# VictoriaMetrics/VictoriaLogs

Hardware: NVIDIA H100
Metric: log rows scanned/sec (LogsQL phrase+regex) (higher is better)
Workload: dtype u8

## Files before the change

### victorialogs_b200/csrc/vl_engine.cu

```cuda
#include <dlfcn.h>
#include <algorithm>
#include <atomic>
#include <chrono>
#include <cmath>
#include <limits>
#include <thread>
#include <cstdio>
#include <cstdlib>
#include <cstring>
#include <functional>
#include <map>
#include <memory>
#include <mutex>
#include "vl_copier.h"
#include "vl_engine.h"
#include "vl_kernels.cuh"
#include "vl_program.h"
#include "vl_part.h"
#include "vl_mathnum.cuh"

using namespace vl;

namespace vl {
static thread_local std::string g_thread_err;
void set_thread_error(const std::string& s) { g_thread_err = s; }
}

struct vlscan_program {
    Program p;
    struct Image { DevBuf leaves, prepass, regexes, blob, u64s, u32s; DevProgram view; };
    std::map<int, std::unique_ptr<Image>> images;
    std::mutex mu;
    const DevProgram& image(int device, cudaStream_t st) {
        std::lock_guard<std::mutex> g(mu);
        auto it = images.find(device);
        if (it != images.end()) return it->second->view;
        auto im = std::make_unique<Image>();
        auto up = [&](DevBuf& b, const void* src, size_t n) { b.ensure(std::max<size_t>(n, 16)); if (n) VL_CUDA(cudaMemcpyAsync(b.p, src, n, cudaMemcpyHostToDevice, st)); };
        up(im->leaves, p.leaves.data(), p.leaves.size() * sizeof(DevLeaf));
        up(im->prepass, p.prepass.data(), p.prepass.size() * sizeof(DevPrepass));
        up(im->regexes, p.regexes.data(), p.regexes.size() * sizeof(DevRegex));
        up(im->blob, p.blob.data(), p.blob.size());
        up(im->u64s, p.u64s.data(), p.u64s.size() * 8);
        up(im->u32s, p.u32s.data(), p.u32s.size() * 4);
        VL_CUDA(cudaStreamSynchronize(st));
        im->view = DevProgram{im->leaves.as<DevLeaf>(), im->prepass.as<DevPrepass>(), im->regexes.as<DevRegex>(), im->blob.as<uint8_t>(), im->u64s.as<uint64_t>(), im->u32s.as<uint32_t>()};
        auto& ref = *im;
        images[device] = std::move(im);
        return ref.view;
    }
    ~vlscan_program() { for (auto& kv : images) { cudaSetDevice(kv.first); kv.second->leaves.release(); kv.second->prepass.release(); kv.second->regexes.release(); kv.second->blob.release(); kv.second->u64s.release(); kv.second->u32s.release(); } }
};

struct vlscan_host_blocks {
    void* pinned = nullptr; size_t bytes = 0;
    std::vector<vlscan_block> blocks;
    std::vector<vlscan_column> cols;
    std::vector<std::string> fields;
    std::vector<std::vector<uint32_t>> dict_offsets;
    std::vector<std::unique_ptr<std::vector<uint8_t>>> owned;
    std::vector<uint64_t> source;
};
struct vlscan_part { vl::part::PartReader r; };

void* vlscan_ctx::ensure_pinned(size_t n) {
    if (n <= pinned_cap) return pinned;
    if (pinned) cudaFreeHost(pinned);
    pinned = nullptr; pinned_cap = 0;
    VL_CUDA(cudaMallocHost(&pinned, n));
    pinned_cap = n;
    return pinned;
}

namespace {

struct ZstdWriter {
    size_t (*compress)(void*, size_t, const void*, size_t, int) = nullptr;
    size_t (*bound)(size_t) = nullptr;
    unsigned (*is_error)(size_t) = nullptr;
    bool ok = false;
    ZstdWriter() {
        void* h = dlopen("libzstd.so.1", RTLD_NOW | RTLD_GLOBAL);
        if (!h) return;
        compress = (decltype(compress))dlsym(h, "ZSTD_compress");
        bound = (decltype(bound))dlsym(h, "ZSTD_compressBound");
        is_error = (decltype(is_error))dlsym(h, "ZSTD_isError");
        ok = compress && bound && is_error;
    }
};
ZstdWriter& zstd_writer() { static ZstdWriter z; return z; }

}

namespace vl {
void finish_batch_layout(vlscan_ctx* ctx, vlscan_batch* b, const std::vector<uint32_t>& rows) {
    b->nblocks = rows.size();
    b->h_rows = rows;
    b->h_word_off.assign(rows.size() + 1, 0);
    b->rows = 0;
    for (size_t i = 0; i < rows.size(); i++) { b->h_word_off[i + 1] = b->h_word_off[i] + (rows[i] + 63) / 64; b->rows += rows[i]; }
    b->nwords = b->h_word_off.back();
    std::vector<uint32_t> wb(b->nwords);
    std::vector<uint64_t> init(b->nwords);
    for (size_t i = 0; i < rows.size(); i++) {
        for (uint64_t w = b->h_word_off[i]; w < b->h_word_off[i + 1]; w++) { wb[w] = (uint32_t)i; init[w] = ~0ull; }
        uint32_t tail = rows[i] & 63;
        if (tail) init[b->h_word_off[i + 1] - 1] = (~0ull) >> (64 - tail);
    }
    b->blk_rows.ensure(std::max<size_t>(rows.size() * 4, 16));
    b->blk_word_off.ensure((rows.size() + 1) * 8);
    b->word_block.ensure(std::max<size_t>(b->nwords * 4, 16));
    b->init_bitmap.ensure(std::max<size_t>(b->nwords * 8, 16));
    if (!rows.empty()) VL_CUDA(cudaMemcpyAsync(b->blk_rows.p, rows.data(), rows.size() * 4, cudaMemcpyHostToDevice, ctx->stream));
    VL_CUDA(cudaMemcpyAsync(b->blk_word_off.p, b->h_word_off.data(), (rows.size() + 1) * 8, cudaMemcpyHostToDevice, ctx->stream));
    if (b->nwords) {
        VL_CUDA(cudaMemcpyAsync(b->word_block.p, wb.data(), b->nwords * 4, cudaMemcpyHostToDevice, ctx->stream));
        VL_CUDA(cudaMemcpyAsync(b->init_bitmap.p, init.data(), b->nwords * 8, cudaMemcpyHostToDevice, ctx->stream));
    }
    VL_CUDA(cudaStreamSynchronize(ctx->stream));
}
}

static uint64_t collect_values_blocks(const vlscan_block* blocks, uint64_t nblocks, std::vector<ZValuesBlock>& zv, const uint8_t* need = nullptr, uint32_t nfields = 0, std::vector<size_t>* at = nullptr) {
    uint64_t zc = 512;
    if (at) at->assign((size_t)nblocks * nfields, SIZE_MAX);
    for (uint64_t b = 0; b < nblocks; b++)
        for (uint32_t k = 0; k < blocks[b].ncols; k++) {
            const vlscan_column& c = blocks[b].cols[k];
            if (c.kind != VLSCAN_COL_VALUES || c.stage != VLSCAN_STAGE_ONDISK) continue;
            if (need && (c.field >= nfields || !need[b * nfields + c.field])) continue;
            if (at && c.field < nfields && (*at)[b * nfields + c.field] == SIZE_MAX) (*at)[b * nfields + c.field] = zv.size();
            zv.push_back({c.values, (size_t)c.values_len, zc});
            zc += c.values_len;
        }
    return zc;
}
static double now_s() { return std::chrono::duration<double>(std::chrono::steady_clock::now().time_since_epoch()).count(); }

namespace {
struct Upload {
    vlscan_ctx* ctx; vlscan_batch* out; const vlscan_block* blocks; uint64_t nblocks; uint32_t nfields; vlscan_stats* stats;
    const std::vector<char>* need_bloom;
    std::vector<DevColumn>& cols = out->h_cols;
    const bool dbg = getenv("VLSCAN_DEBUG_TIMING") != nullptr; const double t_start = now_s();
    Copier io{ctx};
    std::vector<uint32_t> rows = std::vector<uint32_t>(nblocks);
    std::vector<Piece> pieces;
    std::vector<std::unique_ptr<std::vector<uint8_t>>> owned;
    uint64_t cursor = 16;
    ZstdJob zjob;
    uint64_t regen_cursor = 0;
    struct Ondisk { uint64_t col; uint32_t lens_frame, data_frame; uint64_t lens_rel, data_rel; };
    std::vector<Ondisk> ondisk;
    std::vector<OndiskCol> ocols;
    struct TsFrame { uint64_t block; uint32_t frame; uint64_t rel; };
    std::vector<TsFrame> ts_frames;
    std::vector<DevTimestamps> tsv;
    std::vector<ZValuesBlock> zv; std::vector<ZValuesInfo> zinfo; std::vector<size_t> zv_of; std::vector<uint64_t> ts_zoff; size_t zbad = SIZE_MAX; std::string zmsg;
    uint64_t add_piece(const uint8_t* src, uint64_t len) { uint64_t off = arena_reserve(cursor, len); if (len) pieces.push_back({src, len, off}); return off; }
    template <class F> void walk(bool ts, F&& f) {
        for (uint64_t b = 0; b < nblocks; b++) {
            const vlscan_block& blk = blocks[b];
            if (blk.rows > (8u << 20)) throw BadInput("block rows exceed maxRowsPerBlock (8Mi)");
            rows[b] = (uint32_t)blk.rows;
            if (ts) timestamps(blk, b);
            for (uint32_t k = 0; k < blk.ncols; k++) {
                if (blk.cols[k].field >= nfields) throw BadInput("column refers to a field outside the batch field table");
                f(blk, blk.cols[k], (size_t)b * nfields + blk.cols[k].field);
            }
        }
    }
    void sources(const uint8_t* need, bool ts) {
        uint64_t zc = collect_values_blocks(blocks, nblocks, zv, need, nfields, &zv_of);
        for (const ZValuesBlock& v : zv) if (v.n) io.src.push_back({v.p, v.n, v.zoff});
        ts_zoff.resize(ts ? nblocks : 0);
        for (uint64_t b = 0; b < nblocks && ts; b++) {
            const vlscan_block& blk = blocks[b];
            if (blk.ts_marshal_type != MT_ZSTD_NEAREST_DELTA2 && blk.ts_marshal_type != MT_ZSTD_NEAREST_DELTA) continue;
            if (blk.timestamps_len > vl::part::kMaxTimestampsBlockSize) throw BadInput("timestamps block size cannot exceed 8 MiB");
            ts_zoff[b] = zc;
            if (blk.timestamps_len) io.src.push_back({blk.timestamps, blk.timestamps_len, zc});
            zc += blk.timestamps_len;
        }
        if (!io.src.empty()) { ctx->zsrc.ensure(zc + 512); io.send_sources(ctx->zsrc.as<uint8_t>()); }
        zinfo.resize(zv.size());
        const double t_w = now_s();
        if (!zv.empty()) zjob.add_values_blocks(zv.data(), zv.size(), host_threads(), zinfo.data(), &zbad, &zmsg);
        if (dbg) fprintf(stderr, "[vlscan upload] header walk of %zu values blocks on %d host threads: %.1f ms (after %.1f ms of collecting and enqueueing the copies)\n",
                         zv.size(), host_threads(), 1e3 * (now_s() - t_w), 1e3 * (t_w - t_start));
    }
    template <class F> void header(const vlscan_column& c, size_t i, F&& payload) {
        DevColumn& d = cols[i];
        if (d.kind != COL_MISSING) throw BadInput("duplicate column for one field in a block");
        if (c.kind == VLSCAN_COL_CONST) {
            d.kind = COL_CONST; d.meta_len = (uint32_t)c.const_len; d.meta_off = add_piece(c.const_value, c.const_len);
            return;
        }
        if (c.kind != VLSCAN_COL_VALUES) throw BadInput("unknown column kind");
        if (c.value_type < VT_STRING || c.value_type >= VT_MAX) throw BadInput("unknown valueType");
        d.kind = COL_VALUES; d.vt = c.value_type; d.min_value = c.min_value; d.max_value = c.max_value;
        payload();
        if (c.bloom_len % 8) throw BadInput("cannot unmarshal bloomFilter from src with size not multiple by 8");
        if (need_bloom && !(*need_bloom)[c.field]) { d.bloom_words = 0; d.bloom_off = add_piece(c.bloom, 0); }
        else { d.bloom_words = (uint32_t)(c.bloom_len / 8); d.bloom_off = add_piece(c.bloom, c.bloom_len); }
        if (c.value_type == VT_DICT) {
            if (c.dict_len > 8) throw BadInput("valuesDict may contain max 8 items");
            d.dict_len = c.dict_len;
            uint32_t total = c.dict_len ? c.dict_offsets[c.dict_len] : 0;
            d.meta_len = total;
            if (c.dict_len && c.dict_blob == (const uint8_t*)c.dict_offsets + 4 * (c.dict_len + 1)) {
                d.meta_off = add_piece((const uint8_t*)c.dict_offsets, 4 * (c.dict_len + 1) + total);
            } else {
                auto meta = std::make_unique<std::vector<uint8_t>>();
                meta->resize(4 * (c.dict_len + 1) + total);
                if (c.dict_len) memcpy(meta->data(), c.dict_offsets, 4 * (c.dict_len + 1)); else memset(meta->data(), 0, 4);
                if (total) memcpy(meta->data() + 4 * (c.dict_len + 1), c.dict_blob, total);
                d.meta_off = add_piece(meta->data(), meta->size());
                owned.push_back(std::move(meta));
            }
        }
    }
    void values(const vlscan_block& blk, const vlscan_column& c, size_t ci) {
        DevColumn& d = cols[ci];
        if (c.stage == VLSCAN_STAGE_ONDISK) {
            const size_t z = zv_of[ci];
            if (z >= zbad) throw BadInput(zmsg);
            const uint64_t lens_len = zinfo[z].lens_len, data_len = zinfo[z].data_len;
            if (data_len > 0xFFFFFFFFull) throw BadInput("values block too large");
            const uint64_t lr = arena_reserve(regen_cursor, lens_len + 15), dr = arena_reserve(regen_cursor, data_len);
            d.lens_off = lr + 16; d.data_off = dr; d.data_len = data_len;
            ondisk.push_back({ci, (uint32_t)(2 * z), (uint32_t)(2 * z + 1), lr + 15, dr});
            ocols.push_back({ci, lens_len, blk.rows});
        } else if (c.stage == VLSCAN_STAGE_DECODED) {
            const uint8_t* lens_items = c.lens_items; const uint64_t lens_len = c.lens_items_len, data_len = c.data_len;
            if (lens_len < 1) throw BadInput("cannot unmarshal uint64 block type from empty src");
            uint8_t lt = lens_items[0];
            if (lt > 7) throw BadInput("unexpected uint64 block type");
            uint64_t want = lt < 4 ? (blk.rows << lt) : (1ull << (lt - 4));
            if (lens_len - 1 != want) throw BadInput("unexpected block length for uint items");
            d.lens_type = lt;
            if (lt >= 4) { uint64_t v = 0; for (uint64_t i = 0; i < want; i++) v = (v << 8) | lens_items[1 + i]; if (v > 0xFFFFFFFFull) throw BadInput("row length does not fit 32 bits"); d.lens_const = (uint32_t)v; }
            if (data_len > 0xFFFFFFFFull) throw BadInput("values block too large");
            d.lens_off = add_piece(lens_items + 1, lens_len - 1);
            d.data_off = add_piece(c.data, data_len); d.data_len = data_len;
            d.data_const = (blk.rows >= 2 && lt >= 4 && data_len == d.lens_const) ? 1 : 0;
        } else throw BadInput("unknown values stage");
    }
    void timestamps(const vlscan_block& blk, uint64_t b) {
        if (!blk.ts_marshal_type) return;
        if (blk.ts_marshal_type > MT_NEAREST_DELTA) throw BadInput("unknown MarshalType of a timestamps block");
        if (blk.timestamps_len > vl::part::kMaxTimestampsBlockSize) throw BadInput("timestamps block size cannot exceed 8 MiB");
        if (tsv.empty()) { tsv.resize(nblocks); memset(tsv.data(), 0, nblocks * sizeof(DevTimestamps)); }
        DevTimestamps& t = tsv[b];
        t.first = blk.min_timestamp; t.max = blk.max_timestamp;
        if (blk.ts_marshal_type == MT_ZSTD_NEAREST_DELTA2 || blk.ts_marshal_type == MT_ZSTD_NEAREST_DELTA) {
            uint64_t regen = 0; uint32_t id = 0;
            zjob.add_frame(blk.timestamps, blk.timestamps_len, ts_zoff[b], &regen, &id);
            if (regen > 10ull * blk.rows + 16) throw BadInput("cannot unmarshal timestamps: the decompressed block is larger than its varints can be");
            t.mt = blk.ts_marshal_type == MT_ZSTD_NEAREST_DELTA2 ? MT_NEAREST_DELTA2 : MT_NEAREST_DELTA;
            t.len = (uint32_t)regen;
            ts_frames.push_back({b, id, arena_reserve(regen_cursor, regen)});
        } else {
            t.mt = (uint8_t)blk.ts_marshal_type; t.len = (uint32_t)blk.timestamps_len;
            t.off = add_piece(blk.timestamps, blk.timestamps_len);
        }
    }

    uint64_t commit(DevBuf& region, const std::vector<uint64_t>* patch, bool layout) {
        const uint64_t regen_base = (cursor + kArenaAlign - 1) / kArenaAlign * kArenaAlign;
        for (const Ondisk& o : ondisk) {
            DevColumn& d = cols[o.col];
            d.lens_off += regen_base; d.data_off += regen_base;
            zjob.set_dst(o.lens_frame, regen_base + o.lens_rel); zjob.set_dst(o.data_frame, regen_base + o.data_rel);
        }
        for (const TsFrame& tf : ts_frames) { tsv[tf.block].off = regen_base + tf.rel; zjob.set_dst(tf.frame, regen_base + tf.rel); }
        const bool have_z = !ondisk.empty() || !ts_frames.empty();
        if (have_z) cursor = regen_base + regen_cursor;
        const uint64_t bytes = cursor + kArenaPad;
        const double t_desc = now_s();
        region.ensure(bytes);
        const double t_alloc = now_s();
        uint8_t* cols_base = region.as<uint8_t>();
        std::vector<ColPatch> patches;
        if (patch) {
            const uint64_t delta = (uint64_t)(uintptr_t)region.p - (uint64_t)(uintptr_t)out->arena.p;
            cols_base = out->arena.as<uint8_t>();
            patches.resize(patch->size());
            for (size_t i = 0; i < patch->size(); i++) {
                DevColumn& d = cols[(*patch)[i]];
                d.lens_off += delta; d.data_off += delta;
                patches[i].col = (*patch)[i]; patches[i].c = d;
            }
        }
        cudaStream_t cs = ctx->copy_stream;
        cudaEvent_t ev_cleared = io.events.make(), ev_copied = io.events.make();
        VL_CUDA(cudaMemsetAsync(region.p, 0, bytes, ctx->stream));
        VL_CUDA(cudaEventRecord(ev_cleared, ctx->stream));
        VL_CUDA(cudaStreamWaitEvent(cs, ev_cleared, 0));
        const double t_h2d = dbg ? now_s() : 0;
        double t_zrun = 0;
        if (have_z) {
            zjob.set_group_hook([&](uint64_t src_end) { io.wait_sources(ctx->stream, src_end); });
            zjob.run(ctx, ctx->zsrc.as<uint8_t>(), region.as<uint8_t>());
            io.ship_sources(UINT64_MAX);
            if (dbg) t_zrun = now_s();
        }
        io.copy(pieces, region.as<uint8_t>());
        DevBuf& table = patch ? ctx->patch : out->cols;
        const void* entries = patch ? (const void*)patches.data() : (const void*)cols.data();
        const size_t table_bytes = patch ? patches.size() * sizeof(ColPatch) : cols.size() * sizeof(DevColumn);
        table.ensure(std::max<size_t>(table_bytes, 16));
        if (table_bytes) VL_CUDA(cudaMemcpyAsync(table.p, entries, table_bytes, cudaMemcpyHostToDevice, cs));
        io.h2d += table_bytes;
        if (!patch) out->has_ts = !tsv.empty();
        if (!tsv.empty()) {
            out->ts.ensure(nblocks * sizeof(DevTimestamps));
            VL_CUDA(cudaMemcpyAsync(out->ts.p, tsv.data(), nblocks * sizeof(DevTimestamps), cudaMemcpyHostToDevice, cs));
            io.h2d += nblocks * sizeof(DevTimestamps);
        }
        VL_CUDA(cudaEventRecord(ev_copied, cs));
        if (!patches.empty()) {
            VL_CUDA(cudaStreamWaitEvent(ctx->stream, ev_copied, 0));
            k_patch_cols<<<cdiv(patches.size(), 128), 128, 0, ctx->stream>>>(out->cols.as<DevColumn>(), ctx->patch.as<ColPatch>(), (uint32_t)patches.size());
            launch_check(ctx);
        }
        const double t_enq = dbg ? now_s() : 0;
        if (have_z) {
            VL_CUDA(cudaStreamWaitEvent(ctx->stream, ev_copied, 0));
            ctx->zcols.ensure(16 + ocols.size() * sizeof(OndiskCol));
            VL_CUDA(cudaMemsetAsync(ctx->zcols.p, 0, 16, ctx->stream));
            VL_CUDA(cudaMemcpyAsync(ctx->zcols.as<uint8_t>() + 16, ocols.data(), ocols.size() * sizeof(OndiskCol), cudaMemcpyHostToDevice, ctx->stream));
            if (!ocols.empty()) {
                k_finish_ondisk_cols<<<cdiv(ocols.size(), 128), 128, 0, ctx->stream>>>(cols_base, out->cols.as<DevColumn>(), (const OndiskCol*)(ctx->zcols.as<uint8_t>() + 16),
                                                                                         (uint32_t)ocols.size(), ctx->zcols.as<unsigned long long>());
                launch_check(ctx);
            }
            io.h2d += ocols.size() * sizeof(OndiskCol);
            zjob.check(ctx);
            unsigned long long cst[2] = {0, 0};
            VL_CUDA(cudaMemcpy(cst, ctx->zcols.p, 16, cudaMemcpyDeviceToHost));
            static const char* what[] = {"", "cannot unmarshal uint64 block type from empty src", "unexpected uint64 block type", "unexpected block length for uint items", "row length does not fit 32 bits"};
            if (cst[0]) throw BadInput(what[std::min<unsigned long long>(cst[0], 4)]);
        }
        VL_CUDA(cudaStreamWaitEvent(ctx->stream, ev_copied, 0));
        double t_copy = 0;
        if (dbg) { VL_CUDA(cudaStreamSynchronize(ctx->stream)); t_copy = now_s(); }
        if (nfields) out->note_columns(cols);
        if (layout) finish_batch_layout(ctx, out, rows);
        else VL_CUDA(cudaStreamSynchronize(ctx->stream));
        if (dbg) fprintf(stderr, "[vlscan upload] blocks=%llu arena=%.1f MB h2d=%.1f MB pieces=%zu+%zu pinned=%d: describe %.1f ms, alloc %.1f ms, copy %.1f ms (%.1f GB/s), "
                                 "zstd %llu frames / %llu blocks / %llu sequences: enqueue %.1f ms, decode %.1f ms; layout %.1f ms\n", (unsigned long long)nblocks,
                         bytes / 1e6, io.h2d / 1e6, pieces.size(), io.src.size(), (int)io.all_pinned, 1e3 * (t_desc - t_start), 1e3 * (t_alloc - t_desc), 1e3 * (t_enq - (t_zrun > 0 ? t_zrun : t_h2d)), io.h2d / 1e9 / std::max(t_copy - t_start, 1e-9),
                         (unsigned long long)zjob.frames(), (unsigned long long)zjob.compressed_blocks(), (unsigned long long)zjob.sequences(), 1e3 * (t_zrun > 0 ? t_zrun - t_h2d : 0), 1e3 * (t_copy - t_enq), 1e3 * (now_s() - t_copy));
        if (layout) io.h2d += out->nwords * 12 + nblocks * 12;
        if (stats) stats->h2d_bytes += io.h2d;
        return bytes;
    }
};
}

enum UploadMode { UP_FULL = 0, UP_HEADERS = 1, UP_VALUES = 2, UP_LATE = 3 };
static void do_upload(vlscan_ctx* ctx, const char* const* field_names, const size_t* field_name_lens, uint32_t nfields, const vlscan_block* blocks,
                      uint64_t nblocks, vlscan_batch* out, vlscan_stats* stats, const std::vector<char>* need_bloom = nullptr, UploadMode mode = UP_FULL,
                      const uint8_t* need = nullptr, uint64_t* zframes = nullptr) {
    VL_CUDA(cudaSetDevice(ctx->device));
    if (nblocks > 0xFFFFFFF0ull) throw BadInput("too many blocks in one batch");
    out->device = ctx->device; out->nfields = nfields;
    Upload u{ctx, out, blocks, nblocks, nfields, stats, need_bloom};
    if (mode == UP_FULL || mode == UP_HEADERS) {
        for (uint32_t f = 0; f < nfields; f++) out->field_names.emplace_back(field_names[f], field_name_lens[f]);
        u.cols.assign((size_t)nblocks * std::max<uint32_t>(nfields, 1), DevColumn{});
        memset(u.cols.data(), 0, u.cols.size() * sizeof(DevColumn));
        out->late_used = 0; out->split_hdr = mode == UP_HEADERS;
    } else if (u.cols.size() != (size_t)nblocks * std::max<uint32_t>(nfields, 1) || !need) throw BadInput("internal: values phase of a bloom-first upload without its header phase");
    try {
        switch (mode) {
        case UP_FULL:
            u.sources(nullptr, true);
            u.walk(true, [&](const vlscan_block& blk, const vlscan_column& c, size_t i) { u.header(c, i, [&] { u.values(blk, c, i); }); });
            out->arena_bytes = u.commit(out->arena, nullptr, true);
            out->harena_bytes = 0;
            std::vector<DevColumn>().swap(out->h_cols);
            break;
        case UP_HEADERS:
            u.walk(false, [&](const vlscan_block&, const vlscan_column& c, size_t i) {
                u.header(c, i, [&] {
                    if (c.stage != VLSCAN_STAGE_ONDISK && c.stage != VLSCAN_STAGE_DECODED) throw BadInput("unknown values stage");
                    u.cols[i].values_state = VALUES_DEFERRED;
                });
            });
            out->harena_bytes = u.commit(out->harena, nullptr, true);
            break;
        case UP_VALUES:
            u.sources(need, true);
            u.walk(true, [&](const vlscan_block& blk, const vlscan_column& c, size_t i) {
                if (c.kind != VLSCAN_COL_VALUES) return;
                u.cols[i].values_state = need[i] ? VALUES_STAGED : VALUES_ABSENT;
                if (need[i]) u.values(blk, c, i);
            });
            out->arena_bytes = u.commit(out->arena, nullptr, false);
            break;
        case UP_LATE: {
            std::vector<uint64_t> staged;
            u.sources(need, false);
            u.walk(false, [&](const vlscan_block& blk, const vlscan_column& c, size_t i) {
                if (c.kind != VLSCAN_COL_VALUES || !need[i]) return;
                if (u.cols[i].values_state == VALUES_STAGED) throw BadInput("duplicate column for one field in a block");
                u.cols[i].values_state = VALUES_STAGED;
                u.values(blk, c, i);
                staged.push_back(i);
            });
            if (out->late_used == out->late.size()) out->late.emplace_back();
            u.commit(out->late[out->late_used], &staged, false);
            out->late_used++;
            *zframes += u.zjob.frames();
            break;
        }
        }
    } catch (...) {
        cudaStreamSynchronize(ctx->copy_stream); cudaStreamSynchronize(ctx->stream);
        throw;
    }
}

const uint32_t* vl::row_offsets(vlscan_ctx* ctx, const BatchView& B, int slot, const uint32_t* list, const uint32_t* wc, unsigned long long* stats, int wc_slot) {
    uint8_t* ready = ctx->ready[slot].as<uint8_t>();
    if (!ctx->ready_cleared[slot]) { VL_CUDA(cudaMemsetAsync(ready, 0, B.nblocks, ctx->stream)); ctx->ready_cleared[slot] = 1; }
    k_lens_offsets<<<ctx->sm_count * 8, 256, 0, ctx->stream>>>(B, slot, list, wc, ctx->row_off8[slot].as<uint32_t>(), ready, stats, wc_slot); launch_check(ctx);
    return ctx->row_off8[slot].as<uint32_t>();
}

namespace {
struct ScanRun {
    vlscan_ctx* ctx; const vlscan_program* prog; const vlscan_batch* batch;
    DevProgram P; BatchView B; std::vector<int> field_slot;
    unsigned long long* stats;
    size_t regs_used = 0;

    uint64_t* new_reg() {
        if (regs_used == ctx->regs.size()) ctx->regs.emplace_back();
        DevBuf& r = ctx->regs[regs_used++];
        r.ensure(std::max<size_t>(B.nwords * 8, 16));
        return r.as<uint64_t>();
    }
    void free_reg() { regs_used--; }
    void copy_reg(uint64_t* dst, const uint64_t* src) { if (B.nwords) VL_CUDA(cudaMemcpyAsync(dst, src, B.nwords * 8, cudaMemcpyDeviceToDevice, ctx->stream)); }
    void andnot(uint64_t* a, const uint64_t* b) { if (!B.nwords) return; k_andnot<<<cdiv(B.nwords, 256), 256, 0, ctx->stream>>>(a, b, B.nwords); launch_check(ctx); }
    void prepass(const PNode& nd, uint64_t* reg) {
        if (nd.prepass_count == 0) return;
        std::vector<int> slots(nd.prepass_count);
        for (int e = 0; e < nd.prepass_count; e++) slots[e] = field_slot[prog->p.prepass[nd.prepass_begin + e].field];
        size_t off = slots_cursor; slots_cursor += slots.size();
        ctx->slots.ensure(std::max<size_t>(slots_total * 4, 16));
        VL_CUDA(cudaMemcpyAsync(ctx->slots.as<int>() + off, slots.data(), slots.size() * 4, cudaMemcpyHostToDevice, ctx->stream));
        k_prepass<<<cdiv((uint64_t)B.nblocks * 32, 128), 128, 0, ctx->stream>>>(P, B, (uint32_t)nd.prepass_begin, (uint32_t)nd.prepass_count, ctx->slots.as<int>() + off,
                                                                             nd.kind == F_OR, reg, stats);
        launch_check(ctx);
    }
    size_t slots_cursor = 0, slots_total = 0;

    void leaf(int leaf_idx, uint64_t* reg) {
        const DevLeaf& L = prog->p.leaves[leaf_idx];
        if (L.kind == F_NOOP) return;
        int slot = L.field >= 0 ? field_slot[L.field] : -1;
        uint8_t* action = ctx->action.as<uint8_t>(); uint64_t* payload = ctx->payload.as<uint64_t>(); uint64_t* leaf_bm = ctx->leaf_bm.as<uint64_t>();
        uint32_t* lens_blocks = ctx->lens_blocks.as<uint32_t>(); uint32_t* row_blocks = ctx->row_blocks.as<uint32_t>(); uint32_t* wc = ctx->work_count.as<uint32_t>();
        ScanTile* tiles = ctx->tiles.as<ScanTile>();
        VL_CUDA(cudaMemsetAsync(wc, 0, WC_COUNT * 4, ctx->stream));
        if (L.kind == F_EQ_FIELD || L.kind == F_LE_FIELD) {
            const int slot_b = field_slot[L.field2];
            uint32_t* lens_b = ctx->lens_blocks2.as<uint32_t>();
            k_plan_pair<<<cdiv((uint64_t)B.nblocks * 32, 256), 256, 0, ctx->stream>>>(P, B, (uint32_t)leaf_idx, slot, slot_b, reg, action, payload, lens_blocks, lens_b, row_blocks, wc, stats);
            launch_check(ctx);
            if (B.nwords) {
                const int persistent = ctx->sm_count * 8;
                const uint32_t *ro_a = nullptr, *ro_b = nullptr;
                for (int side = 0; side < 2; side++) {
                    const int sl = side ? slot_b : slot;
                    if (sl >= 0) (side ? ro_b : ro_a) = row_offsets(ctx, B, sl, side ? lens_b : lens_blocks, wc, stats, side ? WC_LENS2 : WC_LENS);
                }
                k_row_pair<<<persistent, 256, 0, ctx->stream>>>(P, B, (uint32_t)leaf_idx, slot, slot_b, row_blocks, wc, payload, reg, ro_a, ro_b, leaf_bm, stats); launch_check(ctx);
                k_apply_leaf<<<cdiv(B.nwords, 256), 256, 0, ctx->stream>>>(B, action, leaf_bm, reg); launch_check(ctx);
            }
            return;
        }
        k_plan_leaf<<<cdiv(B.nblocks, VL_PLAN_WARPS), VL_PLAN_WARPS * 32, 0, ctx->stream>>>(P, B, (uint32_t)leaf_idx, slot, reg, action, payload, lens_blocks, row_blocks, tiles, wc, stats);
        launch_check(ctx);
        if (slot >= 0 && B.nwords) {
            const uint32_t vts = batch->slot_vt_mask.empty() ? ~0u : batch->slot_vt_mask[slot];
            const bool has_string = vts >> VT_STRING & 1, has_dict = vts >> VT_DICT & 1;
            const bool has_numeric = (vts & ~((1u << VT_STRING) | (1u << VT_DICT))) != 0;
            const bool may_scan = L.str_strategy == STR_SCAN && has_string;
            const bool may_row = (has_string && L.str_strategy != STR_ALL) || has_numeric;
            const uint32_t* ro = may_scan || may_row ? row_offsets(ctx, B, slot, lens_blocks, wc, stats, WC_LENS) : nullptr;
            if (may_scan) {
                VL_CUDA(cudaMemsetAsync(leaf_bm, 0, B.nwords * 8, ctx->stream));
                ScanParams sp; memset(&sp, 0, sizeof sp);
                sp.mode = L.scan_mode; sp.needle_off = L.scan_needle_off; sp.needle_len = L.scan_needle_len; sp.starts_tok = L.starts_tok; sp.ends_tok = L.ends_tok; sp.regex = L.regex;
                const bool masked = fill_scan_patterns(prog->p.blob.data() + L.scan_needle_off, L.scan_needle_len, sp.pat, sp.msk, sp.delta, sp.nd16);
                if (L.scan_mode == SCAN_CONTAINS || L.scan_mode >= SCAN_RX_DOTPLUS) { sp.starts_tok = sp.ends_tok = 0; }
                auto& evp = next_scan_events();
                VL_CUDA(cudaEventRecord(evp.first, ctx->stream));
                if (masked) k_substr_scan<true><<<ctx->sm_count * ctx->scan_occ[1], VL_SCAN_THREADS, 0, ctx->stream>>>(P, B, slot, sp, tiles, wc, ro, leaf_bm);
                else k_substr_scan<false><<<ctx->sm_count * ctx->scan_occ[0], VL_SCAN_THREADS, 0, ctx->stream>>>(P, B, slot, sp, tiles, wc, ro, leaf_bm);
                launch_check(ctx);
                VL_CUDA(cudaEventRecord(evp.second, ctx->stream));
            }
            if (may_row) { k_row_match<<<ctx->sm_count * ctx->row_occ, 256, 0, ctx->stream>>>(P, B, (uint32_t)leaf_idx, slot, row_blocks, wc, action, payload, reg, ro, leaf_bm); launch_check(ctx); }
            if (has_dict || has_numeric) { k_word_match<<<cdiv(B.nwords, 128), 128, 0, ctx->stream>>>(P, B, (uint32_t)leaf_idx, slot, action, payload, reg, leaf_bm, stats); launch_check(ctx); }
        }
        if (L.kind == F_TIME && B.nwords) {
            ctx->ts_vals.ensure(B.nwords * 64 * 8);
            k_time_match<<<ctx->sm_count * 4, 256, 0, ctx->stream>>>(B, (long long)L.aux0, (long long)L.aux1, row_blocks, wc, ctx->ts_vals.as<unsigned long long>(), leaf_bm, stats);
            launch_check(ctx);
        }
        if (B.nwords) { k_apply_leaf<<<cdiv(B.nwords, 256), 256, 0, ctx->stream>>>(B, action, leaf_bm, reg); launch_check(ctx); }
    }
    std::pair<cudaEvent_t, cudaEvent_t>& next_scan_events() {
        if (ctx->scan_events_used == ctx->scan_events.size()) { cudaEvent_t a, b; VL_CUDA(cudaEventCreate(&a)); VL_CUDA(cudaEventCreate(&b)); ctx->scan_events.emplace_back(a, b); }
        return ctx->scan_events[ctx->scan_events_used++];
    }
    void probe_leaf(int leaf_idx, const uint64_t* reg, uint8_t* need) {
        const DevLeaf& L = prog->p.leaves[leaf_idx];
        if (L.kind == F_NOOP || L.kind == F_TIME) return;
        const int slot = L.field >= 0 ? field_slot[L.field] : -1;
        if (L.kind == F_EQ_FIELD || L.kind == F_LE_FIELD) {
            k_plan_pair<<<cdiv((uint64_t)B.nblocks * 32, 256), 256, 0, ctx->stream>>>(P, B, (uint32_t)leaf_idx, slot, field_slot[L.field2], reg, nullptr, nullptr, nullptr, nullptr, nullptr, nullptr, stats, need);
        } else {
            if (slot < 0) return;
            k_plan_leaf<<<cdiv(B.nblocks, VL_PLAN_WARPS), VL_PLAN_WARPS * 32, 0, ctx->stream>>>(P, B, (uint32_t)leaf_idx, slot, reg, nullptr, nullptr, nullptr, nullptr, nullptr, nullptr, stats, need);
        }
        launch_check(ctx);
    }
    void probe_node(int id, uint64_t* reg, uint8_t* need) {
        const PNode& nd = prog->p.nodes[id];
        switch (nd.kind) {
        case F_NOOP: break;
        case F_AND: case F_OR: {
            uint64_t* r = reg;
            if (nd.prepass_count) { r = new_reg(); copy_reg(r, reg); prepass(nd, r); }
            for (int k : nd.kids) probe_node(k, r, need);
            if (nd.prepass_count) free_reg();
            break;
        }
        case F_NOT: probe_node(nd.kids[0], reg, need); break;
        default: probe_leaf(nd.leaf, reg, need);
        }
    }
    void node(int id, uint64_t* reg) {
        const PNode& nd = prog->p.nodes[id];
        switch (nd.kind) {
        case F_NOOP: break;
        case F_AND: prepass(nd, reg); for (int k : nd.kids) node(k, reg); break;
        case F_OR: {
            prepass(nd, reg);
            uint64_t* res = new_reg(); uint64_t* tmp = new_reg();
            copy_reg(res, reg);
            for (int k : nd.kids) { copy_reg(tmp, res); node(k, tmp); andnot(res, tmp); }
            andnot(reg, res);
            free_reg(); free_reg();
            break;
        }
        case F_NOT: { uint64_t* tmp = new_reg(); copy_reg(tmp, reg); node(nd.kids[0], tmp); andnot(reg, tmp); free_reg(); break; }
        default: leaf(nd.leaf, reg);
        }
    }
};
}

static void read_stats(vlscan_ctx* ctx, vlscan_stats* st, bool check_error) {
    unsigned long long h[ST_COUNT];
    VL_CUDA(cudaMemcpyAsync(h, ctx->stats.p, sizeof h, cudaMemcpyDeviceToHost, ctx->stream));
    VL_CUDA(cudaStreamSynchronize(ctx->stream));
    if (check_error && h[ST_ERROR]) {
        static const char* const msg[] = {"", "cannot unmarshal strings: row lengths do not add up to the data length", "too big index for dict value",
                                          "unexpected length for binary representation of a number", "", "", "the filter needs the timestamps of a block that was handed over without them", "cannot unmarshal timestamps",
                                          "internal: a filter reached the values of a column that the bloom-first probe pass had left on the host"};
        throw BadInput(msg[std::min<unsigned long long>(h[ST_ERROR], 8)]);
    }
    if (!st) return;
    st->values_bytes += h[ST_VALUES_BYTES]; st->bloom_probe_bytes += h[ST_BLOOM_BYTES]; st->columns_read += h[ST_COLUMNS_READ];
    st->bitmap_bytes += h[ST_BITMAP_BYTES]; st->rows_matched += h[ST_ROWS_MATCHED]; st->blocks_matched += h[ST_BLOCKS_MATCHED];
    st->scan_kernel_bytes += h[ST_SCAN_BYTES];
    float ms = 0;
    VL_CUDA(cudaEventElapsedTime(&ms, ctx->ev_begin, ctx->ev_end)); st->gpu_ms += ms;
    for (size_t i = 0; i < ctx->scan_events_used; i++) { VL_CUDA(cudaEventElapsedTime(&ms, ctx->scan_events[i].first, ctx->scan_events[i].second)); st->scan_kernel_ms += ms; }
}

static void do_scan(vlscan_ctx* ctx, const vlscan_program* prog, const vlscan_batch* batch, vlscan_stats* stats) {
    VL_CUDA(cudaSetDevice(ctx->device));
    if (batch->device != ctx->device) throw BadInput("batch lives on another device than the ctx");
    ScanRun run{ctx, prog, batch};
    run.P = const_cast<vlscan_program*>(prog)->image(ctx->device, ctx->stream);
    run.B = batch->view();
    const Program& pr = prog->p;
    run.field_slot.assign(pr.fields.size(), -1);
    for (size_t f = 0; f < pr.fields.size(); f++) for (uint32_t s = 0; s < batch->nfields; s++) if (batch->field_names[s] == pr.fields[f]) run.field_slot[f] = (int)s;
    for (auto& nd : pr.nodes) run.slots_total += nd.prepass_count;
    uint64_t nb = std::max<uint64_t>(batch->nblocks, 1), nw = std::max<uint64_t>(batch->nwords, 1);
    ctx->action.ensure(nb); ctx->payload.ensure(nb * 8); ctx->leaf_bm.ensure(nw * 8);
    ctx->lens_blocks.ensure(nb * 4); ctx->lens_blocks2.ensure(nb * 4); ctx->row_blocks.ensure(nb * 4); ctx->work_count.ensure(WC_COUNT * 4);
    {
        uint64_t max_tiles = batch->arena_bytes / VL_TILE_BYTES + nb + 16;
        ctx->tiles.ensure(max_tiles * sizeof(ScanTile));
    }
    ctx->stats.ensure(ST_COUNT * 8); ctx->totals.ensure(32); ctx->counts.ensure(nb * 4);
    if (ctx->row_off8.size() < batch->nfields) { ctx->row_off8.resize(batch->nfields); ctx->ready.resize(batch->nfields); }
    ctx->ready_cleared.assign(batch->nfields, 0);
    for (uint32_t s = 0; s < batch->nfields; s++) { ctx->row_off8[s].ensure(nw * 32); ctx->ready[s].ensure(nb); }
    uint64_t launches0 = ctx->launches;
    ctx->scan_events_used = 0;
    run.stats = ctx->stats.as<unsigned long long>();
    VL_CUDA(cudaEventRecord(ctx->ev_begin, ctx->stream));
    VL_CUDA(cudaMemsetAsync(ctx->stats.p, 0, ST_COUNT * 8, ctx->stream));
    VL_CUDA(cudaMemsetAsync(ctx->totals.p, 0, 32, ctx->stream));
    uint64_t* reg = run.new_reg();
    run.copy_reg(reg, batch->init_bitmap.as<uint64_t>());
    if (batch->nblocks) {
        run.node(pr.root, reg);
        k_finalize<<<cdiv(batch->nblocks, 8), 256, 0, ctx->stream>>>(run.B, reg, ctx->counts.as<uint32_t>(), run.stats, ctx->totals.as<unsigned long long>());
        launch_check(ctx);
    }
    VL_CUDA(cudaEventRecord(ctx->ev_end, ctx->stream));
    ctx->last_batch = batch; ctx->has_result = true; ctx->kept = false; ctx->last_launches = ctx->launches - launches0;
    ctx->last_nblocks = batch->nblocks; ctx->last_nwords = batch->nwords; ctx->last_rows = batch->rows;
    if (stats) {
        read_stats(ctx, stats, true);
        stats->blocks += batch->nblocks; stats->rows += batch->rows; stats->gpu_launches += ctx->launches - launches0;
    }
}

static void do_probe(vlscan_ctx* ctx, const vlscan_program* prog, const vlscan_batch* batch, std::vector<uint8_t>& need) {
    VL_CUDA(cudaSetDevice(ctx->device));
    ScanRun run{ctx, prog, batch};
    run.P = const_cast<vlscan_program*>(prog)->image(ctx->device, ctx->stream);
    run.B = batch->view();
    const Program& pr = prog->p;
    run.field_slot.assign(pr.fields.size(), -1);
    for (size_t f = 0; f < pr.fields.size(); f++) for (uint32_t s = 0; s < batch->nfields; s++) if (batch->field_names[s] == pr.fields[f]) run.field_slot[f] = (int)s;
    for (auto& nd : pr.nodes) run.slots_total += nd.prepass_count;
    const size_t cells = (size_t)batch->nblocks * batch->nfields;
    need.assign(cells, 0);
    if (!cells || !batch->nwords) return;
    ctx->need.ensure(std::max<size_t>(cells, 16)); ctx->stats.ensure(ST_COUNT * 8);
    VL_CUDA(cudaMemsetAsync(ctx->need.p, 0, cells, ctx->stream));
    VL_CUDA(cudaMemsetAsync(ctx->stats.p, 0, ST_COUNT * 8, ctx->stream));
    run.stats = ctx->stats.as<unsigned long long>();
    uint64_t* reg = run.new_reg();
    run.copy_reg(reg, batch->init_bitmap.as<uint64_t>());
    run.probe_node(pr.root, reg, ctx->need.as<uint8_t>());
    VL_CUDA(cudaMemcpyAsync(need.data(), ctx->need.p, cells, cudaMemcpyDeviceToHost, ctx->stream));
    VL_CUDA(cudaStreamSynchronize(ctx->stream));
}

extern "C" {

int vlscan_device_count(void) {
    int n = 0;
    if (cudaGetDeviceCount(&n) != cudaSuccess) { cudaGetLastError(); return 0; }
    return n;
}

vlscan_ctx* vlscan_ctx_create(int device) {
    vlscan_ctx* ctx = new vlscan_ctx();
    int rc = guarded(nullptr, [&] {
        int n = vlscan_device_count();
        if (n <= 0) throw CudaFail("no CUDA device is available: libvlscan has no CPU fallback", 100);
        ctx->device = ((device % n) + n) % n;
        VL_CUDA(cudaSetDevice(ctx->device));
        VL_CUDA(cudaStreamCreateWithFlags(&ctx->stream, cudaStreamNonBlocking));
        VL_CUDA(cudaStreamCreateWithFlags(&ctx->copy_stream, cudaStreamNonBlocking));
        VL_CUDA(cudaEventCreate(&ctx->ev_begin)); VL_CUDA(cudaEventCreate(&ctx->ev_end));
        cudaDeviceProp prop; VL_CUDA(cudaGetDeviceProperties(&prop, ctx->device)); ctx->sm_count = prop.multiProcessorCount;
        VL_CUDA(cudaOccupancyMaxActiveBlocksPerMultiprocessor(&ctx->scan_occ[0], k_substr_scan<false>, VL_SCAN_THREADS, 0));
        VL_CUDA(cudaOccupancyMaxActiveBlocksPerMultiprocessor(&ctx->scan_occ[1], k_substr_scan<true>, VL_SCAN_THREADS, 0));
        for (int& o : ctx->scan_occ) o = std::max(o, 1);
        VL_CUDA(cudaOccupancyMaxActiveBlocksPerMultiprocessor(&ctx->row_occ, k_row_match, 256, 0));
        ctx->row_occ = std::max(ctx->row_occ, 1);
    });
    if (rc) { delete ctx; return nullptr; }
    return ctx;
}
void vlscan_ctx_free(vlscan_ctx* ctx) {
    if (!ctx) return;
    cudaSetDevice(ctx->device);
    if (ctx->copy_stream) cudaStreamSynchronize(ctx->copy_stream);
    if (ctx->stream) cudaStreamSynchronize(ctx->stream);
    for (DevBuf* b : {&ctx->action, &ctx->payload, &ctx->leaf_bm, &ctx->lens_blocks, &ctx->row_blocks, &ctx->work_count, &ctx->stats, &ctx->totals, &ctx->counts, &ctx->slots, &ctx->hit_offs, &ctx->hits, &ctx->tiles, &ctx->lens_blocks2}) b->release();
    for (auto& r : ctx->regs) r.release();
    for (auto& r : ctx->row_off8) r.release();
    for (auto& r : ctx->ready) r.release();
    ctx->zsrc.release(); ctx->zcols.release(); ctx->ztest.release(); ctx->ts_vals.release();
    for (DevBuf* b : {&ctx->hit_block, &ctx->glens, &ctx->goffs, &ctx->gtiles, &ctx->gout, &ctx->gstat, &ctx->hslot, &ctx->hblk, &ctx->htab, &ctx->hgrp, &ctx->lcand, &ctx->ftab, &ctx->patch, &ctx->unstaged}) b->release();
    for (DevBuf& b : ctx->ftxt) b.release();
    zstd_dev_free(ctx->zdev);
    delete ctx->pool;
    if (ctx->pinned) cudaFreeHost(ctx->pinned);
    delete ctx->recycle;
    for (auto& e : ctx->scan_events) { cudaEventDestroy(e.first); cudaEventDestroy(e.second); }
    if (ctx->ev_begin) cudaEventDestroy(ctx->ev_begin);
    if (ctx->ev_end) cudaEventDestroy(ctx->ev_end);
    if (ctx->copy_stream) cudaStreamDestroy(ctx->copy_stream);
    if (ctx->stream) cudaStreamDestroy(ctx->stream);
    delete ctx;
}
const char* vlscan_last_error(const vlscan_ctx* ctx) { return ctx ? ctx->err.c_str() : g_thread_err.c_str(); }
void* vlscan_ctx_stream(const vlscan_ctx* ctx) { return (void*)ctx->stream; }
int vlscan_ctx_sync(vlscan_ctx* ctx) { return guarded(ctx, [&] { VL_CUDA(cudaSetDevice(ctx->device)); VL_CUDA(cudaStreamSynchronize(ctx->stream)); }); }

int vlscan_program_create(const void* tree, size_t tree_len, vlscan_program** out) {
    *out = nullptr;
    auto* pg = new vlscan_program();
    int rc = guarded(nullptr, [&] { ProgramBuilder(tree, tree_len, pg->p).build(); });
    if (rc) { delete pg; return rc; }
    *out = pg;
    return 0;
}
void vlscan_program_free(vlscan_program* prog) { delete prog; }
uint32_t vlscan_program_nfields(const vlscan_program* prog) { return (uint32_t)prog->p.fields.size(); }
const char* vlscan_program_field(const vlscan_program* prog, uint32_t i, size_t* len) { if (i >= prog->p.fields.size()) { *len = 0; return nullptr; } *len = prog->p.fields[i].size(); return prog->p.fields[i].data(); }
int64_t vlscan_program_leaf_tokens(const vlscan_program* prog, uint32_t leaf, char* buf, size_t cap) {
    if (leaf >= prog->p.leaf_tokens.size()) return -1;
    std::string s; for (size_t i = 0; i < prog->p.leaf_tokens[leaf].size(); i++) { if (i) s.push_back('\n'); s += prog->p.leaf_tokens[leaf][i]; }
    if (s.size() > cap) return -1;
    memcpy(buf, s.data(), s.size());
    return (int64_t)s.size();
}

int vlscan_eval_predicate(int kind, const void* value, size_t value_len, const void* arg1, size_t arg1_len, const void* arg2, size_t arg2_len, uint64_t aux0, uint64_t aux1) {
    if (value_len > 0xFFFFFFFFull || arg1_len > 0xFFFFFFFFull || arg2_len > 0xFFFFFFFFull) return -1;
    const uint8_t* v = (const uint8_t*)value; const uint32_t vn = (uint32_t)value_len;
    const uint8_t* a = (const uint8_t*)arg1; const uint32_t an = (uint32_t)arg1_len;
    switch (kind) {
    case F_REGEXP: {
        try { return vl::compile_regex(std::string((const char*)a, an)).match(v, vn) ? 1 : 0; } catch (const vl::RxError& e) { vl::set_thread_error(e.what()); return -2; }
    }
    case 14: return vl::any_case_match(v, vn, a, an, false) ? 1 : 0;
    case 15: return vl::any_case_match(v, vn, a, an, true) ? 1 : 0;
    case 16: return vl::match_sequence(v, vn, vl::PhraseList{a, an}) ? 1 : 0;
    case 17: return vl::match_all_phrases(v, vn, vl::PhraseList{a, an}) ? 1 : 0;
    case 18: return vl::match_any_phrase(v, vn, vl::PhraseList{a, an}) ? 1 : 0;
    }
    if (kind < F_EXACT_PREFIX || kind > F_IPV4_RANGE) return -1;
    return vl::range_predicate(kind, (const uint8_t*)value, (uint32_t)value_len, (const uint8_t*)arg1, (uint32_t)arg1_len, (const uint8_t*)arg2, (uint32_t)arg2_len, aux0, aux1) ? 1 : 0;
}

int64_t vlscan_program_prepass_tokens(const vlscan_program* prog, char* buf, size_t cap) {
    const Program& P = prog->p;
    std::string s;
    for (const PNode& nd : P.nodes) {
        if (nd.kind != F_AND && nd.kind != F_OR) continue;
        s += nd.kind == F_AND ? "A" : "O";
        for (int k = 0; k < nd.prepass_count; k++) {
            const DevPrepass& pp = P.prepass[(size_t)nd.prepass_begin + k];
            s += "\t" + P.fields[pp.field];
            const uint32_t* offs = (const uint32_t*)(P.blob.data() + pp.tok_offs_off);
            for (uint32_t t = 0; t < pp.ntokens; t++) { s += "\x1f"; s.append((const char*)P.blob.data() + pp.tok_blob_off + offs[t], offs[t + 1] - offs[t]); }
        }
        s += "\n";
    }
    if (s.size() > cap) return -1;
    memcpy(buf, s.data(), s.size());
    return (int64_t)s.size();
}

int64_t vlscan_program_in_hashes(const vlscan_program* prog, uint32_t leaf, uint64_t* out, size_t cap) {
    const Program& P = prog->p;
    if (leaf >= P.leaves.size() || P.leaves[leaf].kind != F_IN) return -1;
    const DevLeaf& L = P.leaves[leaf];
    std::vector<uint64_t> v;
    v.push_back(L.nhashes); v.insert(v.end(), P.u64s.begin() + L.hashes_off, P.u64s.begin() + L.hashes_off + L.nhashes);
    if (L.in_skip_sets) v.push_back(UINT64_MAX);
    else {
        v.push_back(L.in_nsets);
        for (uint32_t k = 0; k < L.in_nsets; k++) {
            const uint32_t off = P.u32s[L.in_sets_off + 2 * k], n = P.u32s[L.in_sets_off + 2 * k + 1];
            v.push_back(n); v.insert(v.end(), P.u64s.begin() + off, P.u64s.begin() + off + n);
        }
    }
    if (v.size() > cap) return -1;
    memcpy(out, v.data(), v.size() * 8);
    return (int64_t)v.size();
}

int64_t vlscan_program_in_typed(const vlscan_program* prog, uint32_t leaf, int value_type, uint64_t* out, size_t cap) {
    const Program& P = prog->p;
    if (leaf >= P.leaves.size() || P.leaves[leaf].kind != F_IN || value_type < VT_UINT8 || value_type >= VT_MAX) return -1;
    const DevLeaf& L = P.leaves[leaf];
    const uint32_t n = L.in_typed_cnt[value_type];
    if (n > cap) return -1;
    if (n) memcpy(out, P.u64s.data() + L.in_typed_off[value_type], (size_t)n * 8);
    return (int64_t)n;
}

int vlscan_parse_typed(int value_type, const void* s, size_t len, uint64_t* out) {
    const std::string v((const char*)s, len);
    uint64_t u = 0; int64_t i = 0; double f = 0; uint32_t ip = 0;
    switch (value_type) {
    case VT_UINT8: case VT_UINT16: case VT_UINT32: case VT_UINT64: if (!vl::parse_u64(v, &u)) return 0; *out = u; return 1;
    case VT_INT64: if (!vl::parse_i64(v, &i)) return 0; *out = (uint64_t)i; return 1;
    case VT_FLOAT64: if (!vl::parse_f64_exact(v, &f)) return 0; memcpy(out, &f, 8); return 1;
    case VT_IPV4: if (!vl::parse_ipv4(v, &ip)) return 0; *out = ip; return 1;
    case VT_ISO8601: if (!vl::parse_iso8601(v, &i)) return 0; *out = (uint64_t)i; return 1;
    }
    return -1;
}

double vlscan_parse_math_number(const void* s, size_t len) {
    if (len > 0xFFFFFFFFull) return NAN;
    return vl::mn::parse_math_number((const uint8_t*)s, (uint32_t)len);
}

int vlscan_format_float64(uint64_t ieee_bits, char* buf, size_t cap) {
    uint8_t tmp[VL_FMT_F64_MAX];
    int n = vl::fmt_f64(tmp, ieee_bits);
    if ((size_t)n > cap) return -1;
    memcpy(buf, tmp, (size_t)n);
    return n;
}

int vlscan_batch_upload(vlscan_ctx* ctx, const char* const* field_names, const size_t* field_name_lens, uint32_t nfields, const vlscan_block* blocks,
                        uint64_t nblocks, vlscan_batch** out, vlscan_stats* stats) {
    *out = nullptr;
    auto* b = new vlscan_batch();
    int rc = guarded(ctx, [&] { do_upload(ctx, field_names, field_name_lens, nfields, blocks, nblocks, b, stats); });
    if (rc) { delete b; return rc; }
    *out = b;
    return 0;
}
void vlscan_batch_free(vlscan_batch* batch) { delete batch; }
uint64_t vlscan_batch_nblocks(const vlscan_batch* b) { return b->nblocks; }
uint64_t vlscan_batch_rows(const vlscan_batch* b) { return b->rows; }
uint64_t vlscan_batch_words(const vlscan_batch* b) { return b->nwords; }
uint64_t vlscan_batch_device_bytes(const vlscan_batch* b) { return b->device_bytes(); }

int vlscan_batch_download(vlscan_ctx* ctx, const vlscan_batch* batch, vlscan_host_blocks** out) {
    *out = nullptr;
    auto* hb = new vlscan_host_blocks();
    int rc = guarded(ctx, [&] {
        VL_CUDA(cudaSetDevice(ctx->device));
        if (batch->split_hdr) throw BadInput("a batch staged bloom-first cannot be downloaded");
        hb->bytes = batch->arena_bytes;
        VL_CUDA(cudaMallocHost(&hb->pinned, std::max<size_t>(hb->bytes, 16)));
        std::vector<DevColumn> cols((size_t)batch->nblocks * batch->nfields);
        VL_CUDA(cudaMemcpyAsync(hb->pinned, batch->arena.p, hb->bytes, cudaMemcpyDeviceToHost, ctx->stream));
        if (!cols.empty()) VL_CUDA(cudaMemcpyAsync(cols.data(), batch->cols.p, cols.size() * sizeof(DevColumn), cudaMemcpyDeviceToHost, ctx->stream));
        VL_CUDA(cudaStreamSynchronize(ctx->stream));
        hb->fields = batch->field_names;
        const uint8_t* base = (const uint8_t*)hb->pinned;
        hb->blocks.resize(batch->nblocks);
        hb->cols.reserve(cols.size());
        std::vector<size_t> first(batch->nblocks + 1, 0);
        for (uint64_t b = 0; b < batch->nblocks; b++) {
            first[b] = hb->cols.size();
            for (uint32_t f = 0; f < batch->nfields; f++) {
                const DevColumn& d = cols[(size_t)b * batch->nfields + f];
                if (d.kind == COL_MISSING) continue;
                vlscan_column c; memset(&c, 0, sizeof c);
                c.field = f;
                if (d.kind == COL_CONST) { c.kind = VLSCAN_COL_CONST; c.const_value = base + d.meta_off; c.const_len = d.meta_len; hb->cols.push_back(c); continue; }
                c.kind = VLSCAN_COL_VALUES; c.value_type = d.vt; c.stage = VLSCAN_STAGE_DECODED; c.dict_len = d.dict_len; c.min_value = d.min_value; c.max_value = d.max_value;
                uint64_t items = d.lens_type < 4 ? ((uint64_t)batch->h_rows[b] << d.lens_type) : (1ull << (d.lens_type - 4));
                uint8_t* tb = (uint8_t*)hb->pinned + d.lens_off - 1;
                *tb = d.lens_type;
                c.lens_items = tb; c.lens_items_len = items + 1;
                c.data = base + d.data_off; c.data_len = d.data_len;
                c.bloom = base + d.bloom_off; c.bloom_len = (uint64_t)d.bloom_words * 8;
                if (d.vt == VT_DICT) { c.dict_offsets = (const uint32_t*)(base + d.meta_off); c.dict_blob = base + d.meta_off + 4 * (d.dict_len + 1); }
                hb->cols.push_back(c);
            }
        }
        first[batch->nblocks] = hb->cols.size();
        for (uint64_t b = 0; b < batch->nblocks; b++) { hb->blocks[b].rows = batch->h_rows[b]; hb->blocks[b].ncols = (uint32_t)(first[b + 1] - first[b]); hb->blocks[b].cols = hb->cols.data() + first[b]; }
        if (batch->has_ts && batch->nblocks) {
            std::vector<DevTimestamps> ts(batch->nblocks);
            VL_CUDA(cudaMemcpy(ts.data(), batch->ts.p, ts.size() * sizeof(DevTimestamps), cudaMemcpyDeviceToHost));
            for (uint64_t b = 0; b < batch->nblocks; b++) {
                if (!ts[b].mt) continue;
                vlscan_block& blk = hb->blocks[b];
                blk.ts_marshal_type = ts[b].mt; blk.timestamps = base + ts[b].off; blk.timestamps_len = ts[b].len;
                blk.min_timestamp = ts[b].first; blk.max_timestamp = ts[b].max;
            }
        }
    });
    if (rc) { if (hb->pinned) cudaFreeHost(hb->pinned); delete hb; return rc; }
    *out = hb;
    return 0;
}
static void marshal_bytes_block(std::vector<uint8_t>& dst, const uint8_t* src, size_t n) {
    if (n < 128) { dst.push_back(0); dst.push_back((uint8_t)n); dst.insert(dst.end(), src, src + n); return; }
    ZstdWriter& z = zstd_writer();
    if (!z.ok) throw BadInput("libzstd.so.1 is not available for compressing values blocks");
    int level = n <= 512 ? 1 : n <= 4096 ? 2 : 3;
    size_t cap = z.bound(n), old = dst.size();
    dst.push_back(1);
    dst.resize(old + 1 + 10 + cap);
    size_t got = z.compress(dst.data() + old + 11, cap, src, n, level);
    if (z.is_error(got)) throw BadInput("ZSTD_compress failed");
    uint8_t vu[10]; int k = 0; uint64_t v = got; while (v >= 0x80) { vu[k++] = (uint8_t)(v | 0x80); v >>= 7; } vu[k++] = (uint8_t)v;
    memcpy(dst.data() + old + 1, vu, k);
    memmove(dst.data() + old + 1 + k, dst.data() + old + 11, got);
    dst.resize(old + 1 + k + got);
}

int vlscan_host_blocks_compress(const vlscan_host_blocks* in, int threads, vlscan_host_blocks** out) {
    *out = nullptr;
    auto* hb = new vlscan_host_blocks();
    int rc = guarded(nullptr, [&] {
        const size_t ncols = in->cols.size();
        std::vector<std::vector<uint8_t>> packed(ncols);
        std::atomic<size_t> next{0}; std::atomic<bool> failed{false}; std::string fail_msg; std::mutex mu;
        auto work = [&] {
            for (;;) {
                size_t i0 = next.fetch_add(64); if (i0 >= ncols || failed) return;
                for (size_t i = i0; i < std::min(ncols, i0 + 64); i++) {
                    const vlscan_column& c = in->cols[i];
                    if (c.kind != VLSCAN_COL_VALUES) continue;
                    try {
                        if (c.stage == VLSCAN_STAGE_ONDISK) packed[i].assign(c.values, c.values + c.values_len);
                        else { marshal_bytes_block(packed[i], c.lens_items, c.lens_items_len); marshal_bytes_block(packed[i], c.data, c.data_len); }
                    } catch (const BadInput& e) { std::lock_guard<std::mutex> g(mu); fail_msg = e.msg; failed = true; return; }
                }
            }
        };
        int nt = threads > 0 ? threads : (int)std::max(1u, std::thread::hardware_concurrency());
        std::vector<std::thread> pool; for (int t = 1; t < nt; t++) pool.emplace_back(work);
        work(); for (auto& t : pool) t.join();
        if (failed) throw BadInput(fail_msg);
        uint64_t cursor = 16, vbytes = 0;
        std::vector<uint64_t> off_a(ncols, 0), off_b(ncols, 0), off_v(ncols, 0);
        for (size_t i = 0; i < ncols; i++) {
            const vlscan_column& c = in->cols[i];
            if (c.kind == VLSCAN_COL_CONST) { off_a[i] = arena_reserve(cursor, c.const_len); continue; }
            off_a[i] = arena_reserve(cursor, c.bloom_len);
            if (c.value_type == VT_DICT) off_b[i] = arena_reserve(cursor, 4 * (c.dict_len + 1) + (c.dict_len ? c.dict_offsets[c.dict_len] : 0));
            off_v[i] = vbytes; vbytes += packed[i].size();
        }
        const uint64_t vbase = (cursor + kArenaPad + 63) / 64 * 64;
        hb->bytes = vbase + vbytes + 64;
        VL_CUDA(cudaMallocHost(&hb->pinned, hb->bytes));
        uint8_t* base = (uint8_t*)hb->pinned;
        memset(base, 0, vbase);
        hb->fields = in->fields; hb->cols = in->cols; hb->blocks = in->blocks;
        for (size_t i = 0; i < ncols; i++) {
            vlscan_column& c = hb->cols[i];
            if (c.kind == VLSCAN_COL_CONST) { if (c.const_len) memcpy(base + off_a[i], c.const_value, c.const_len); c.const_value = base + off_a[i]; continue; }
            if (c.bloom_len) memcpy(base + off_a[i], c.bloom, c.bloom_len);
            c.bloom = base + off_a[i];
            if (c.value_type == VT_DICT) {
                uint32_t total = c.dict_len ? c.dict_offsets[c.dict_len] : 0;
                uint8_t* m = base + off_b[i];
                if (c.dict_len) memcpy(m, c.dict_offsets, 4 * (c.dict_len + 1)); else memset(m, 0, 4);
                if (total) memcpy(m + 4 * (c.dict_len + 1), c.dict_blob, total);
                c.dict_offsets = (const uint32_t*)m; c.dict_blob = m + 4 * (c.dict_len + 1);
            }
            memcpy(base + vbase + off_v[i], packed[i].data(), packed[i].size());
            c.stage = VLSCAN_STAGE_ONDISK; c.values = base + vbase + off_v[i]; c.values_len = packed[i].size();
            c.lens_items = nullptr; c.lens_items_len = 0; c.data = nullptr; c.data_len = 0;
            std::vector<uint8_t>().swap(packed[i]);
        }
        size_t k = 0;
        for (size_t b = 0; b < hb->blocks.size(); b++) { hb->blocks[b].cols = hb->cols.data() + k; k += hb->blocks[b].ncols; }
    });
    if (rc) { if (hb->pinned) cudaFreeHost(hb->pinned); delete hb; return rc; }
    *out = hb;
    return 0;
}

int vlscan_zstd_inspect(const void* bytes_block, size_t len, uint64_t out[5]) {
    return guarded(nullptr, [&] {
        ZstdJob job;
        uint64_t regen = 0; uint32_t id = 0;
        size_t used = job.add_bytes_block((const uint8_t*)bytes_block, len, 512, &regen, &id);
        out[0] = used; out[1] = regen; out[2] = job.blocks(); out[3] = job.compressed_blocks(); out[4] = job.sequences();
    });
}

int vlscan_zstd_walk_digest(const vlscan_block* blocks, uint64_t nblocks, int threads, uint64_t out[12]) {
    return guarded(nullptr, [&] {
        std::vector<ZValuesBlock> zv;
        collect_values_blocks(blocks, nblocks, zv);
        std::vector<ZValuesInfo> info(zv.size());
        ZstdJob job; size_t bad = SIZE_MAX; std::string msg;
        const double t0 = now_s();
        if (!zv.empty()) job.add_values_blocks(zv.data(), zv.size(), threads, info.data(), &bad, &msg);
        const double t1 = now_s();
        if (bad != SIZE_MAX) throw BadInput("values block " + std::to_string(bad) + ": " + msg);
        job.prepare();
        const double t2 = now_s();
        job.digest(out);
        uint64_t h = 5; for (const ZValuesInfo& x : info) { h = (h ^ x.lens_len) * 0x9E3779B97F4A7C15ull; h = (h ^ x.data_len) * 0x9E3779B97F4A7C15ull; h ^= h >> 29; }
        out[0] ^= h;
        out[4] = job.frames(); out[5] = job.blocks(); out[6] = job.groups(); out[7] = job.compressed_blocks(); out[8] = job.sequences();
        out[9] = (uint64_t)((t1 - t0) * 1e9); out[10] = (uint64_t)((t2 - t1) * 1e9); out[11] = 0;
    });
}

static void zstd_decompress_frames(vlscan_ctx* ctx, uint32_t nframes, const void* const* frames, const size_t* frame_lens, void* dst, const uint64_t* dst_offsets) {
    {
        VL_CUDA(cudaSetDevice(ctx->device));
        ZstdJob job;
        std::vector<uint8_t> packed(512, 0);
        for (uint32_t i = 0; i < nframes; i++) {
            uint64_t regen = 0; uint32_t id = 0;
            job.add_frame((const uint8_t*)frames[i], frame_lens[i], packed.size(), &regen, &id);
            if (regen != dst_offsets[i + 1] - dst_offsets[i]) throw BadInput("cannot decompress block: frame content size differs from the destination size");
            job.set_dst(id, 16 + dst_offsets[i]);
            packed.insert(packed.end(), (const uint8_t*)frames[i], (const uint8_t*)frames[i] + frame_lens[i]);
        }
        const uint64_t total = nframes ? dst_offsets[nframes] : 0;
        ctx->zsrc.ensure(packed.size() + 512); ctx->ztest.ensure(16 + total + 64);
        VL_CUDA(cudaMemcpyAsync(ctx->zsrc.p, packed.data(), packed.size(), cudaMemcpyHostToDevice, ctx->stream));
        VL_CUDA(cudaMemsetAsync(ctx->ztest.p, 0xA5, 16 + total + 64, ctx->stream));
        job.run(ctx, ctx->zsrc.as<uint8_t>(), ctx->ztest.as<uint8_t>());
        job.check(ctx);
        if (total) VL_CUDA(cudaMemcpy(dst, ctx->ztest.as<uint8_t>() + 16, total, cudaMemcpyDeviceToHost));
    }
}

int vlscan_zstd_decompress(vlscan_ctx* ctx, uint32_t nframes, const void* const* frames, const size_t* frame_lens, void* dst, const uint64_t* dst_offsets) {
    return guarded(ctx, [&] { zstd_decompress_frames(ctx, nframes, frames, frame_lens, dst, dst_offsets); });
}

int vlscan_part_open(vlscan_ctx* ctx, const char* path, vlscan_inflate_fn inflate, void* user, vlscan_part** out) {
    *out = nullptr;
    auto* p = new vlscan_part();
    int rc = guarded(ctx, [&] {
        if (!inflate && !ctx) throw BadInput("vlscan_part_open needs a ctx (device ZSTD decoder) or an inflate callback");
        vl::part::Inflate inf;
        if (inflate) inf = [&](const uint8_t* f, size_t n, uint8_t* dst, size_t dn) { if (inflate(user, f, n, dst, dn) != 0) throw BadInput("the inflate callback failed on a metadata frame of the part"); };
        else inf = [&](const uint8_t* f, size_t n, uint8_t* dst, size_t dn) { const void* fr[1] = {f}; const size_t ln[1] = {n}; const uint64_t offs[2] = {0, dn}; zstd_decompress_frames(ctx, 1, fr, ln, dst, offs); };
        p->r.open(path, inf);
    });
    if (rc) { delete p; return rc; }
    *out = p;
    return 0;
}
void vlscan_part_free(vlscan_part* part) { delete part; }
void vlscan_part_header(const vlscan_part* part, uint64_t out[8]) {
    const vl::part::PartHeader& h = part->r.ph;
    out[0] = h.FormatVersion; out[1] = h.CompressedSizeBytes; out[2] = h.UncompressedSizeBytes; out[3] = h.RowsCount; out[4] = h.BlocksCount;
    out[5] = (uint64_t)h.MinTimestamp; out[6] = (uint64_t)h.MaxTimestamp; out[7] = h.BloomValuesShardsCount;
}
uint64_t vlscan_part_nblocks(const vlscan_part* part) { return part->r.blockHeaders.size(); }
int vlscan_part_block_header(const vlscan_part* part, uint64_t i, uint64_t out[15]) {
    return guarded(nullptr, [&] {
        if (i >= part->r.blockHeaders.size()) throw BadInput("block index outside the part");
        const vl::part::BlockHeader& b = part->r.blockHeaders[i];
        out[0] = b.sid.accountID; out[1] = b.sid.projectID; out[2] = b.sid.hi; out[3] = b.sid.lo; out[4] = b.uncompressedSizeBytes; out[5] = b.rowsCount;
        out[6] = b.tsOffset; out[7] = b.tsSize; out[8] = (uint64_t)b.minTimestamp; out[9] = (uint64_t)b.maxTimestamp; out[10] = b.tsMarshalType;
        out[11] = b.chIndexOffset; out[12] = b.chIndexSize; out[13] = b.chOffset; out[14] = b.chSize;
    });
}
int vlscan_part_timestamps(const vlscan_part* part, uint64_t i, const uint8_t** data, uint64_t* len) {
    return guarded(nullptr, [&] {
        if (i >= part->r.blockHeaders.size()) throw BadInput("block index outside the part");
        const vl::part::BlockHeader& b = part->r.blockHeaders[i];
        if (b.tsSize > vl::part::kMaxTimestampsBlockSize) throw BadInput("timestamps block size is too big");
        *data = part->r.timestamps_file().at(b.tsOffset, b.tsSize, "a timestamps block"); *len = b.tsSize;
    });
}
uint32_t vlscan_part_ncolumn_names(const vlscan_part* part) { return (uint32_t)part->r.columnNames.size(); }
const char* vlscan_part_column_name(const vlscan_part* part, uint32_t i, size_t* len) { if (i >= part->r.columnNames.size()) { *len = 0; return nullptr; } const std::string& s = part->r.columnNames[i]; *len = s.size(); return s.data(); }
int vlscan_part_blocks(const vlscan_part* part, const char* const* field_names, const size_t* field_name_lens, uint32_t nfields, uint64_t block_lo, uint64_t block_hi,
                       int64_t min_timestamp, int64_t max_timestamp, vlscan_host_blocks** out) {
    *out = nullptr;
    auto* hb = new vlscan_host_blocks();
    int rc = guarded(nullptr, [&] {
        std::vector<std::string> fields;
        for (uint32_t f = 0; f < nfields; f++) { std::string n(field_names[f], field_name_lens[f]); fields.push_back(n.empty() ? "_msg" : n); }
        for (size_t a = 0; a < fields.size(); a++) for (size_t b = a + 1; b < fields.size(); b++) if (fields[a] == fields[b]) throw BadInput("duplicate field name");
        vl::part::Described d;
        part->r.describe(fields, block_lo, block_hi, min_timestamp, max_timestamp, d);
        hb->fields = std::move(d.fields); hb->cols = std::move(d.cols); hb->blocks = std::move(d.blocks); hb->owned = std::move(d.owned); hb->source = std::move(d.source);
        for (const vlscan_column& c : hb->cols) hb->bytes += c.const_len + c.values_len + c.bloom_len;
    });
    if (rc) { delete hb; return rc; }
    *out = hb;
    return 0;
}
const uint64_t* vlscan_host_blocks_source(const vlscan_host_blocks* hb, uint64_t* n) { *n = hb->source.size(); return hb->source.data(); }

const vlscan_block* vlscan_host_blocks_get(const vlscan_host_blocks* hb, uint64_t* nblocks, uint32_t* nfields) { *nblocks = hb->blocks.size(); *nfields = (uint32_t)hb->fields.size(); return hb->blocks.data(); }
const char* vlscan_host_blocks_field(const vlscan_host_blocks* hb, uint32_t i, size_t* len) { if (i >= hb->fields.size()) { *len = 0; return nullptr; } *len = hb->fields[i].size(); return hb->fields[i].data(); }
uint64_t vlscan_host_blocks_bytes(const vlscan_host_blocks* hb) { return hb->bytes; }
void vlscan_host_blocks_free(vlscan_host_blocks* hb) { if (!hb) return; if (hb->pinned) cudaFreeHost(hb->pinned); delete hb; }

int vlscan_scan_resident(vlscan_ctx* ctx, const vlscan_program* prog, const vlscan_batch* batch, vlscan_stats* stats) {
    return guarded(ctx, [&] { do_scan(ctx, prog, batch, stats); });
}

int vlscan_last_scan_stats(vlscan_ctx* ctx, vlscan_stats* stats) {
    return guarded(ctx, [&] {
        if (!ctx->has_result) throw BadInput("no scan on this ctx yet");
        VL_CUDA(cudaSetDevice(ctx->device));
        read_stats(ctx, stats, true);
        stats->blocks += ctx->last_nblocks; stats->rows += ctx->last_rows; stats->gpu_launches += ctx->last_launches;
    });
}

int vlscan_fetch_results(vlscan_ctx* ctx, uint64_t* out_bitmap_words, uint32_t* out_match_counts, vlscan_stats* stats) {
    return guarded(ctx, [&] {
        if (!ctx->has_result) throw BadInput("no scan result to fetch on this ctx");
        VL_CUDA(cudaSetDevice(ctx->device));
        uint64_t d2h = 0;
        if (out_bitmap_words && ctx->last_nwords) { VL_CUDA(cudaMemcpyAsync(out_bitmap_words, ctx->regs[0].p, ctx->last_nwords * 8, cudaMemcpyDeviceToHost, ctx->stream)); d2h += ctx->last_nwords * 8; }
        if (out_match_counts && ctx->last_nblocks) { VL_CUDA(cudaMemcpyAsync(out_match_counts, ctx->counts.p, ctx->last_nblocks * 4, cudaMemcpyDeviceToHost, ctx->stream)); d2h += ctx->last_nblocks * 4; }
        read_stats(ctx, nullptr, true);
        if (stats) stats->d2h_bytes += d2h;
    });
}

int vlscan_result_digest(vlscan_ctx* ctx, uint64_t block_lo, uint64_t block_hi, uint64_t key_base, uint64_t* out_digest) {
    return guarded(ctx, [&] {
        if (!ctx->has_result) throw BadInput("no scan result on this ctx");
        if (block_lo > block_hi || block_hi > ctx->last_nblocks) throw BadInput("block range outside the batch of the last scan");
        VL_CUDA(cudaSetDevice(ctx->device));
        ctx->hit_offs.ensure(16);
        VL_CUDA(cudaMemsetAsync(ctx->hit_offs.p, 0, 8, ctx->stream));
        if (block_hi > block_lo) {
            k_bitmap_digest<<<cdiv(block_hi - block_lo, 128), 128, 0, ctx->stream>>>(ctx->last_batch->view(), ctx->regs[0].as<uint64_t>(), (uint32_t)block_lo, (uint32_t)block_hi, key_base, ctx->hit_offs.as<unsigned long long>());
            launch_check(ctx);
        }
        VL_CUDA(cudaMemcpyAsync(out_digest, ctx->hit_offs.p, 8, cudaMemcpyDeviceToHost, ctx->stream));
        VL_CUDA(cudaStreamSynchronize(ctx->stream));
    });
}

int vlscan_totals_sum(vlscan_ctx* const* ctxs, int nctx, uint64_t out4[4]) {
    out4[0] = out4[1] = out4[2] = out4[3] = 0;
    for (int i = 0; i < nctx; i++) {
        vlscan_ctx* ctx = ctxs[i];
        int rc = guarded(ctx, [&] {
            if (!ctx->has_result) throw BadInput("no scan result on this ctx");
            VL_CUDA(cudaSetDevice(ctx->device));
            unsigned long long t[4];
            VL_CUDA(cudaMemcpyAsync(t, ctx->totals.p, 32, cudaMemcpyDeviceToHost, ctx->stream));
            VL_CUDA(cudaStreamSynchronize(ctx->stream));
            for (int k = 0; k < 4; k++) out4[k] += t[k];
        });
        if (rc) return rc;
    }
    return 0;
}

int vlscan_result_device_ptrs(vlscan_ctx* ctx, void** bitmap_words, void** match_counts, void** totals4) {
    if (!ctx->has_result) { ctx->err = "no scan result on this ctx"; return -1; }
    if (bitmap_words) *bitmap_words = ctx->regs[0].p;
    if (match_counts) *match_counts = ctx->counts.p;
    if (totals4) *totals4 = ctx->totals.p;
    return 0;
}

static vlscan_batch::CellSig cell_sig(const vlscan_column& c) {
    vlscan_batch::CellSig g;
    g.stage = c.stage;
    if (c.stage == VLSCAN_STAGE_ONDISK) g.len0 = c.values_len; else { g.len0 = c.lens_items_len; g.len1 = c.data_len; }
    return g;
}

static int scan_batch_impl(vlscan_ctx* ctx, const vlscan_program* prog, const char* const* field_names, const size_t* field_name_lens, uint32_t nfields,
                           const vlscan_block* blocks, uint64_t nblocks, uint64_t* out_bitmap_words, uint32_t* out_match_counts, vlscan_stats* stats, bool keep) {
    vlscan_batch* b = ctx->recycle ? ctx->recycle : new vlscan_batch();
    ctx->recycle = nullptr;
    b->field_names.clear(); b->slot_vt_mask.clear();
    uint64_t launches0 = ctx->launches;
    std::vector<char> need_bloom(nfields, 0), in_prog(nfields, 0);
    {
        const Program& P = prog->p;
        auto mark = [&](std::vector<char>& m, int field) { for (uint32_t s = 0; s < nfields; s++) if (std::string(field_names[s], field_name_lens[s]) == P.fields[field]) m[s] = 1; };
        for (const DevLeaf& L : P.leaves) if (L.nhashes || L.nhashes2 || L.in_nsets) mark(need_bloom, L.field);
        for (const DevPrepass& pp : P.prepass) if (pp.nhashes) mark(need_bloom, pp.field);
        if (keep) for (size_t f = 0; f < P.fields.size(); f++) mark(in_prog, (int)f);
    }
    int bf = 1;
    if (const char* e = getenv("VLSCAN_BLOOM_FIRST")) bf = atoi(e);
    bool probes = false;
    for (char c : need_bloom) probes |= c != 0;
    if (ctx->bf_prog != (const void*)prog) { ctx->bf_prog = prog; ctx->bf_skip = 0; }
    const bool probe = bf != 0 && probes && nblocks > 0 && (bf == 2 || ctx->bf_skip == 0);
    if (!probe && ctx->bf_skip > 0) ctx->bf_skip--;
    int rc;
    if (probe || keep) {
        rc = guarded(ctx, [&] {
            do_upload(ctx, field_names, field_name_lens, nfields, blocks, nblocks, b, stats, &need_bloom, UP_HEADERS);
            std::vector<uint8_t> need;
            if (probe) do_probe(ctx, prog, b, need);
            else {
                need.assign(std::max<size_t>((size_t)nblocks * nfields, 1), 0);
                for (uint64_t i = 0; i < nblocks; i++)
                    for (uint32_t k = 0; k < blocks[i].ncols; k++) if (blocks[i].cols[k].field < nfields && in_prog[blocks[i].cols[k].field]) need[i * nfields + blocks[i].cols[k].field] = 1;
            }
            uint64_t vals_all = 0, vals_need = 0, cols_all = 0, cols_need = 0;
            for (uint64_t i = 0; i < nblocks; i++)
                for (uint32_t k = 0; k < blocks[i].ncols; k++) {
                    const vlscan_column& c = blocks[i].cols[k];
                    if (c.kind != VLSCAN_COL_VALUES || c.field >= nfields) continue;
                    const bool needed = need[i * nfields + c.field] != 0;
                    cols_all++; cols_need += needed;
                    if (keep && !in_prog[c.field]) continue;
                    const uint64_t n = c.stage == VLSCAN_STAGE_ONDISK ? c.values_len : c.lens_items_len + c.data_len;
                    vals_all += n;
                    if (needed) vals_need += n;
                }
            if (stats && probe) { stats->staged_columns += cols_need; stats->pruned_columns += cols_all - cols_need; }
            if (probe && vals_need * 8 > vals_all * 7) ctx->bf_skip = 7;
            do_upload(ctx, field_names, field_name_lens, nfields, blocks, nblocks, b, stats, &need_bloom, UP_VALUES, need.data());
            if (keep) {
                b->h_sig.assign((size_t)nblocks * nfields, vlscan_batch::CellSig{});
                b->h_ncols.resize(nblocks);
                for (uint64_t i = 0; i < nblocks; i++) {
                    b->h_ncols[i] = blocks[i].ncols;
                    for (uint32_t k = 0; k < blocks[i].ncols; k++) {
                        const vlscan_column& c = blocks[i].cols[k];
                        if (c.kind == VLSCAN_COL_VALUES) b->h_sig[i * nfields + c.field] = cell_sig(c);
                    }
                }
            }
        });
    } else rc = guarded(ctx, [&] { do_upload(ctx, field_names, field_name_lens, nfields, blocks, nblocks, b, stats, &need_bloom); });
    if (!rc) rc = vlscan_scan_resident(ctx, prog, b, nullptr);
    if (!rc) rc = vlscan_fetch_results(ctx, out_bitmap_words, out_match_counts, stats);
    if (!rc && stats) {
        rc = guarded(ctx, [&] { read_stats(ctx, stats, true); stats->blocks += b->nblocks; stats->rows += b->rows; stats->gpu_launches += ctx->launches - launches0; });
    }
    if (keep && !rc) ctx->kept = true;
    else { ctx->has_result = false; ctx->last_batch = nullptr; ctx->kept = false; }
    ctx->recycle = b;
    return rc;
}

int vlscan_scan_batch(vlscan_ctx* ctx, const vlscan_program* prog, const char* const* field_names, const size_t* field_name_lens, uint32_t nfields,
                      const vlscan_block* blocks, uint64_t nblocks, uint64_t* out_bitmap_words, uint32_t* out_match_counts, vlscan_stats* stats) {
    return scan_batch_impl(ctx, prog, field_names, field_name_lens, nfields, blocks, nblocks, out_bitmap_words, out_match_counts, stats, false);
}

int vlscan_scan_batch_keep(vlscan_ctx* ctx, const vlscan_program* prog, const char* const* field_names, const size_t* field_name_lens, uint32_t nfields,
                           const vlscan_block* blocks, uint64_t nblocks, uint64_t* out_bitmap_words, uint32_t* out_match_counts, vlscan_stats* stats) {
    if (!ctx || !prog) return guarded(nullptr, [&] { throw BadInput(!ctx ? "vlscan_scan_batch_keep needs a vlscan_ctx on a CUDA device (there is no CPU fallback)" : "vlscan_scan_batch_keep: no program"); });
    return scan_batch_impl(ctx, prog, field_names, field_name_lens, nfields, blocks, nblocks, out_bitmap_words, out_match_counts, stats, true);
}

int vlscan_stage_selected(vlscan_ctx* ctx, const vlscan_block* blocks, uint64_t nblocks, const char* const* field_names, const size_t* field_name_lens, uint32_t nfields,
                          const uint32_t* block_list, uint64_t nlist, uint64_t out_info[4]) {
    uint64_t info[4] = {0, 0, 0, 0};
    bool staging = false;
    const int rc = guarded(ctx, [&] {
        if (nfields == 0) throw BadInput("vlscan_stage_selected needs at least one field");
        const std::vector<std::string> names = canonical_names(field_names, field_name_lens, nfields, "vlscan_stage_selected");
        if (nlist && !block_list) throw BadInput("vlscan_stage_selected: block list missing");
        if (!ctx) throw BadInput("vlscan_stage_selected needs a vlscan_ctx on a CUDA device (there is no CPU fallback)");
        if (!ctx->has_result || !ctx->kept || !ctx->recycle || ctx->last_batch != ctx->recycle) throw BadInput("no kept scan on this ctx (vlscan_scan_batch_keep keeps one until the next scan)");
        vlscan_batch* b = ctx->recycle;
        VL_CUDA(cudaSetDevice(ctx->device));
        const uint32_t nf = b->nfields;
        std::vector<char> want(nf, 0);
        for (const std::string& n : names) {
            const int slot = b->field_slot(n);
            if (slot < 0) throw BadInput("field `" + n + "` is not a field of the kept batch");
            want[slot] = 1;
        }
        if (!blocks || nblocks != b->nblocks) throw BadInput("the block descriptors differ from those of the kept scan: " + std::to_string(nblocks) + " blocks instead of " + std::to_string(b->nblocks));
        std::vector<uint8_t> sel(nblocks, 0);
        if (block_list) {
            for (uint64_t i = 0; i < nlist; i++) {
                if (block_list[i] >= nblocks) throw BadInput("block_list[" + std::to_string(i) + "] = " + std::to_string(block_list[i]) + " is outside the kept batch of " + std::to_string(nblocks) + " blocks");
                sel[block_list[i]] = 1;
            }
        } else if (nblocks) {
            std::vector<uint32_t> cnt(nblocks);
            VL_CUDA(cudaMemcpyAsync(cnt.data(), ctx->counts.p, nblocks * 4, cudaMemcpyDeviceToHost, ctx->stream));
            VL_CUDA(cudaStreamSynchronize(ctx->stream));
            for (uint64_t i = 0; i < nblocks; i++) sel[i] = cnt[i] != 0;
        }
        auto mismatch = [&](uint64_t i, const char* what) { return BadInput("the block descriptors differ from those of the kept scan: block " + std::to_string(i) + ", " + what); };
        for (uint64_t i = 0; i < nblocks; i++) {
            if (!sel[i]) continue;
            const vlscan_block& blk = blocks[i];
            if (blk.rows != b->h_rows[i]) throw mismatch(i, "row count");
            if (blk.ncols != b->h_ncols[i] || (blk.ncols && !blk.cols)) throw mismatch(i, "column count");
            for (uint32_t k = 0; k < blk.ncols; k++) {
                const vlscan_column& c = blk.cols[k];
                if (c.field >= nf) throw mismatch(i, "field of a column");
                const DevColumn& d = b->h_cols[i * nf + c.field];
                if (c.kind == VLSCAN_COL_CONST) { if (d.kind != COL_CONST || d.meta_len != c.const_len) throw mismatch(i, "const column"); }
                else if (c.kind == VLSCAN_COL_VALUES) {
                    if (d.kind != COL_VALUES || d.vt != c.value_type) throw mismatch(i, "column kind or value type");
                    const vlscan_batch::CellSig want = cell_sig(c), &had = b->h_sig[i * nf + c.field];
                    if (had.stage != want.stage || had.len0 != want.len0 || had.len1 != want.len1) throw mismatch(i, "values stage or payload lengths");
                } else throw mismatch(i, "column kind");
            }
        }
        std::vector<uint8_t> need((size_t)nblocks * nf, 0);
        for (uint64_t i = 0; i < nblocks; i++) {
            if (!sel[i]) continue;
            for (uint32_t s = 0; s < nf; s++) {
                const DevColumn& d = b->h_cols[i * nf + s];
                if (!want[s] || d.kind != COL_VALUES) continue;
                if (d.values_state == VALUES_STAGED) info[1]++;
                else { need[i * nf + s] = 1; info[0]++; }
            }
        }
        if (!info[0]) return;
        vlscan_stats st;
        memset(&st, 0, sizeof st);
        staging = true;
        do_upload(ctx, nullptr, nullptr, nf, blocks, nblocks, b, &st, nullptr, UP_LATE, need.data(), &info[3]);
        info[2] = st.h2d_bytes;
    });
    if (rc && staging) {
        ctx->has_result = false; ctx->last_batch = nullptr; ctx->kept = false;
        info[0] = info[1] = info[2] = info[3] = 0;
    }
    if (out_info && !rc) memcpy(out_info, info, sizeof info);
    return rc;
}

}
```

### victorialogs_b200/csrc/vl_engine.h

```cpp
#pragma once
#include <cuda_runtime.h>
#include <stdint.h>
#include <algorithm>
#include <string>
#include <vector>
#include "../../include/vlscan.h"
#include "vl_types.h"
#include "vl_zstd.h"
#include "vl_zstd_walk.h"
#include "vl_hostpool.h"

namespace vl {

void set_thread_error(const std::string& s);
#define VL_CUDA(call)                                                                                                   \
    do {                                                                                                                \
        cudaError_t e__ = (call);                                                                                       \
        if (e__ != cudaSuccess) throw CudaFail(std::string(#call) + ": " + cudaGetErrorString(e__), (int)e__);        \
    } while (0)
struct CudaFail { std::string msg; int code; CudaFail(std::string m, int c) : msg(std::move(m)), code(c) {} };

struct DevBuf {
    void* p = nullptr; size_t cap = 0;
    void ensure(size_t n) {
        if (n <= cap) return;
        if (p) VL_CUDA(cudaFree(p));
        p = nullptr; cap = 0;
        size_t want = n + std::min<size_t>(n / 8, (size_t)256 << 20) + 256;
        VL_CUDA(cudaMalloc(&p, want)); cap = want;
    }
    void release() { if (p) cudaFree(p); p = nullptr; cap = 0; }
    template <class T> T* as() const { return (T*)p; }
};



static const size_t kArenaAlign = 16;
static const size_t kArenaPad = 32;
inline uint64_t arena_reserve(uint64_t& cursor, uint64_t len) {
    uint64_t off = (cursor + kArenaAlign - 1) / kArenaAlign * kArenaAlign;
    cursor = off + len + kArenaPad;
    return off;
}

}

struct vlscan_batch {
    int device = 0;
    uint32_t nfields = 0;
    std::vector<std::string> field_names;
    uint64_t nblocks = 0, nwords = 0, rows = 0;
    uint64_t arena_bytes = 0, harena_bytes = 0;
    vl::DevBuf arena, cols, blk_rows, blk_word_off, word_block, init_bitmap, ts;
    vl::DevBuf harena;
    bool split_hdr = false;
    std::vector<vl::DevColumn> h_cols;
    bool has_ts = false;
    std::vector<uint32_t> h_rows;
    std::vector<uint64_t> h_word_off;
    std::vector<uint32_t> slot_vt_mask;
    std::vector<vl::DevBuf> late;
    size_t late_used = 0;
    struct CellSig { uint64_t len0 = 0, len1 = 0; uint32_t stage = 0; };
    std::vector<CellSig> h_sig;
    std::vector<uint32_t> h_ncols;
    void note_columns(const std::vector<vl::DevColumn>& cols) {
        slot_vt_mask.assign(nfields, 0);
        for (size_t i = 0; i < cols.size(); i++) if (cols[i].kind == vl::COL_VALUES) slot_vt_mask[i % nfields] |= 1u << cols[i].vt;
    }
    int field_slot(const std::string& name) const {
        for (uint32_t s = 0; s < nfields; s++) if (field_names[s] == name) return (int)s;
        return -1;
    }
    vl::BatchView view() const {
        vl::BatchView v;
        v.arena = arena.as<uint8_t>(); v.hdr = split_hdr ? harena.as<uint8_t>() : arena.as<uint8_t>(); v.cols = cols.as<vl::DevColumn>(); v.blk_rows = blk_rows.as<uint32_t>();
        v.blk_word_off = blk_word_off.as<uint64_t>(); v.word_block = word_block.as<uint32_t>();
        v.ts = has_ts ? ts.as<vl::DevTimestamps>() : nullptr;
        v.nblocks = (uint32_t)nblocks; v.nfields = nfields; v.nwords = nwords;
        return v;
    }
    uint64_t device_bytes() const {
        uint64_t n = arena.cap + harena.cap + cols.cap + blk_rows.cap + blk_word_off.cap + word_block.cap + init_bitmap.cap + ts.cap;
        for (const vl::DevBuf& r : late) n += r.cap;
        return n;
    }
    ~vlscan_batch() {
        cudaSetDevice(device); arena.release(); harena.release(); cols.release(); blk_rows.release(); blk_word_off.release(); word_block.release(); init_bitmap.release(); ts.release();
        for (vl::DevBuf& r : late) r.release();
    }
};

struct vlscan_ctx {
    int device = 0;
    cudaStream_t stream = nullptr;
    cudaStream_t copy_stream = nullptr;
    std::string err;
    uint64_t launches = 0;
    vl::DevBuf action, payload, leaf_bm, lens_blocks, work_count, stats, totals, counts, slots, tiles;
    vl::DevBuf lens_blocks2;
    vl::DevBuf row_blocks;
    vl::DevBuf hit_offs, hits;
    std::vector<vl::DevBuf> regs;
    std::vector<vl::DevBuf> row_off8;
    std::vector<vl::DevBuf> ready;
    std::vector<char> ready_cleared;
    vl::DevBuf hit_block, glens, goffs, gtiles, gout, gstat;
    vl::DevBuf ts_vals;
    vl::DevBuf hslot;
    vl::DevBuf hblk, htab, hgrp;
    vl::DevBuf lcand;
    vl::DevBuf ftab;
    std::vector<vl::DevBuf> ftxt;
    vl::DevBuf need;
    const void* bf_prog = nullptr; int bf_skip = 0;
    vl::DevBuf zsrc, zcols, ztest;
    vl::ZstdDev* zdev = nullptr;
    void* pinned = nullptr; size_t pinned_cap = 0;
    vl::HostPool* pool = nullptr;
    cudaEvent_t ev_begin = nullptr, ev_end = nullptr;
    std::vector<std::pair<cudaEvent_t, cudaEvent_t>> scan_events; size_t scan_events_used = 0;
    const vlscan_batch* last_batch = nullptr;
    uint64_t last_nblocks = 0, last_nwords = 0, last_rows = 0;
    vlscan_batch* recycle = nullptr;
    bool kept = false;
    vl::DevBuf patch, unstaged;
    bool has_result = false;
    uint64_t last_launches = 0;
    int sm_count = 132;
    int scan_occ[2] = {1, 1};
    int row_occ = 1;
    void* ensure_pinned(size_t n);
};

namespace vl {
void finish_batch_layout(vlscan_ctx* ctx, vlscan_batch* b, const std::vector<uint32_t>& rows);

const uint32_t* row_offsets(vlscan_ctx* ctx, const BatchView& B, int slot, const uint32_t* list, const uint32_t* wc, unsigned long long* stats, int wc_slot);

template <class F> int guarded(vlscan_ctx* ctx, F&& f) {
    try { f(); return 0; }
    catch (const CudaFail& e) { set_thread_error(e.msg); if (ctx) ctx->err = e.msg; return e.code > 0 ? e.code : 1; }
    catch (const BadInput& e) { set_thread_error(e.msg); if (ctx) ctx->err = e.msg; return -1; }
    catch (const ProgError& e) { set_thread_error(e.what()); if (ctx) ctx->err = e.what(); return -2; }
    catch (const std::exception& e) { set_thread_error(e.what()); if (ctx) ctx->err = e.what(); return -3; }
}

inline void launch_check(vlscan_ctx* ctx) { ctx->launches++; VL_CUDA(cudaGetLastError()); }
inline unsigned cdiv(uint64_t a, uint64_t b) { return (unsigned)((a + b - 1) / b); }

inline std::vector<std::string> canonical_names(const char* const* names, const size_t* lens, uint32_t n, const char* what) {
    if (n && (!names || !lens)) throw BadInput(std::string(what) + ": field names missing");
    std::vector<std::string> out;
    for (uint32_t f = 0; f < n; f++) out.push_back(lens[f] ? std::string(names[f], lens[f]) : "_msg");
    return out;
}
}
```

### victorialogs_b200/csrc/vl_gen.cu

```cuda
#include <algorithm>
#include <cstring>
#include <vector>
#include "vl_engine.h"
#include "vl_hd.cuh"

using namespace vl;

namespace {

__host__ __device__ inline uint64_t gen_rnd(uint64_t seed, uint64_t b, uint64_t i, uint64_t k) {
    uint64_t z = seed + (b + 1) * 0x9E3779B97F4A7C15ULL + (i + 1) * 0xD1B54A32D192ED03ULL + (k + 1) * 0x8CB92BA72F3D8DD7ULL;
    z ^= z >> 30; z *= 0xBF58476D1CE4E5B9ULL; z ^= z >> 27; z *= 0x94D049BB133111EBULL; z ^= z >> 31;
    return z;
}

__device__ const char* const D_VOCAB[12] = {"error", "timeout", "GET /api/v1/items", "conn 10.0.0.7 refused", "errors", "timeouts", "GETS /api/v2",
                                            "connection refuse", "conn reset by peer", "terror", "error timeout", "POST /api/v1/items"};
__device__ const char* const D_LEVELS[8] = {"debug", "info", "warn", "error", "fatal", "ERROR", "FATAL", "INFO"};
__device__ const uint32_t D_STATUS[9] = {200, 201, 204, 301, 400, 404, 500, 502, 503};

__device__ __forceinline__ int put_str(uint8_t* d, const char* s) { int n = 0; while (s[n]) { d[n] = (uint8_t)s[n]; n++; } return n; }
__device__ __forceinline__ int put_hex(uint8_t* d, uint64_t v, int width) { for (int i = width - 1; i >= 0; i--) { uint32_t x = v & 15; d[i] = (uint8_t)(x < 10 ? '0' + x : 'a' + x - 10); v >>= 4; } return width; }

__device__ int gen_msg(const vlscan_gen_config& c, bool hot, uint64_t b, uint64_t i, uint8_t* d) {
    uint64_t r0 = gen_rnd(c.seed, b, i, 0);
    int n = 0;
    const uint32_t focus = (c.columns_mask >> 8) & 15;
    if (hot && (r0 % 1000) < c.hit_row_permille) n += put_str(d + n, D_VOCAB[focus ? focus - 1 : (r0 >> 32) % 12]); else n += put_str(d + n, "message");
    n += put_str(d + n, " for the stream "); n += fmt_u64(d + n, b);
    n += put_str(d + n, " and worker "); n += fmt_u64(d + n, b % 7);
    n += put_str(d + n, "; ip="); n += fmt_ipv4(d + n, (uint32_t)gen_rnd(c.seed, b, i, 1));
    uint64_t ua = gen_rnd(c.seed, b, i, 2), ub = gen_rnd(c.seed, b, i, 3);
    n += put_str(d + n, "; uuid=");
    n += put_hex(d + n, ua & 0xffffffffULL, 8); d[n++] = '-'; n += put_hex(d + n, (ua >> 32) & 0xffff, 4); d[n++] = '-'; n += put_hex(d + n, ua >> 48, 4); d[n++] = '-';
    n += put_hex(d + n, ub & 0xffff, 4); d[n++] = '-'; n += put_hex(d + n, ub >> 16, 12);
    n += put_str(d + n, "; u64="); n += fmt_u64(d + n, gen_rnd(c.seed, b, i, 4));
    return n;
}
__device__ int gen_path(const vlscan_gen_config& c, uint64_t b, uint64_t i, uint8_t* d) {
    uint64_t r = gen_rnd(c.seed, b, i, 6);
    int n = 0;
    switch (r % 4) {
    case 0: case 1: n += put_str(d, "api/v1/items/"); n += fmt_u64(d + n, (r >> 8) % 100000); break;
    case 2: n += put_str(d, "static/js/app."); n += fmt_u64(d + n, (r >> 8) % 1000); n += put_str(d + n, ".js"); break;
    default: n += put_str(d, "health");
    }
    return n;
}

struct GenInfo {
    uint32_t msg_bytes, msg_minlen, msg_maxlen, msg_tokens;
    uint32_t path_bytes, path_minlen, path_maxlen, path_tokens, path_distinct;
    uint32_t level_first[8];
    uint32_t status_mask;
    uint32_t overflow;
};

__device__ bool set_insert(unsigned long long* tab, uint32_t cap_mask, uint64_t key, uint32_t* overflow) {
    if (key == 0) key = 0x9E3779B97F4A7C15ULL;
    uint32_t slot = (uint32_t)(key * 0x9E3779B97F4A7C15ULL >> 32) & cap_mask;
    for (uint32_t probes = 0; probes <= cap_mask; probes++) {
        unsigned long long prev = atomicCAS(&tab[slot], 0ull, (unsigned long long)key);
        if (prev == 0ull) return true;
        if (prev == key) return false;
        slot = (slot + 1) & cap_mask;
    }
    atomicExch(overflow, 1u);
    return false;
}
template <class F> __device__ void ascii_tokens(const uint8_t* s, int n, F&& f) {
    int i = 0;
    while (i < n) {
        while (i < n && !is_token_char(s[i])) i++;
        int st = i;
        while (i < n && is_token_char(s[i])) i++;
        if (i > st) f(s + st, (uint32_t)(i - st));
    }
}

__global__ void k_gen_measure(vlscan_gen_config c, uint64_t block_lo, uint32_t nblocks, GenInfo* __restrict__ info, unsigned long long* __restrict__ tables, uint32_t cap_mask) {
    __shared__ GenInfo s;
    unsigned long long* tab_msg = tables + (size_t)blockIdx.x * 3 * (cap_mask + 1);
    unsigned long long* tab_path = tab_msg + (cap_mask + 1);
    unsigned long long* tab_vals = tab_path + (cap_mask + 1);
    for (uint32_t j = blockIdx.x; j < nblocks; j += gridDim.x) {
        uint64_t b = block_lo + j;
        uint64_t lo = b * c.rows_per_block, hi = min((unsigned long long)c.total_rows, (unsigned long long)(lo + c.rows_per_block));
        uint32_t rows = (uint32_t)(hi - lo);
        for (uint32_t k = threadIdx.x; k < 3 * (cap_mask + 1); k += blockDim.x) tab_msg[k] = 0;
        if (threadIdx.x == 0) { memset(&s, 0, sizeof s); s.msg_minlen = s.path_minlen = 0xFFFFFFFFu; for (int k = 0; k < 8; k++) s.level_first[k] = 0xFFFFFFFFu; }
        __syncthreads();
        bool hot = gen_rnd(c.seed, b, 0xFFFFFFFFULL, 0) % 1000 < c.hot_block_permille;
        uint8_t buf[192];
        for (uint32_t i = threadIdx.x; i < rows; i += blockDim.x) {
            if (c.columns_mask & 1) {
                int n = gen_msg(c, hot, b, i, buf);
                atomicAdd(&s.msg_bytes, (uint32_t)n); atomicMin(&s.msg_minlen, (uint32_t)n); atomicMax(&s.msg_maxlen, (uint32_t)n);
                ascii_tokens(buf, n, [&](const uint8_t* t, uint32_t tl) { if (set_insert(tab_msg, cap_mask, xxh64(t, tl), &s.overflow)) atomicAdd(&s.msg_tokens, 1u); });
            }
            if (c.columns_mask & 2) atomicMin(&s.level_first[gen_rnd(c.seed, b, i, 5) % 8], i);
            if (c.columns_mask & 4) {
                int n = gen_path(c, b, i, buf);
                atomicAdd(&s.path_bytes, (uint32_t)n); atomicMin(&s.path_minlen, (uint32_t)n); atomicMax(&s.path_maxlen, (uint32_t)n);
                if (set_insert(tab_vals, cap_mask, xxh64(buf, (uint32_t)n), &s.overflow)) atomicAdd(&s.path_distinct, 1u);
                ascii_tokens(buf, n, [&](const uint8_t* t, uint32_t tl) { if (set_insert(tab_path, cap_mask, xxh64(t, tl), &s.overflow)) atomicAdd(&s.path_tokens, 1u); });
            }
            if (c.columns_mask & 8) atomicOr(&s.status_mask, 1u << (gen_rnd(c.seed, b, i, 7) % 9));
        }
        __syncthreads();
        if (threadIdx.x == 0) info[j] = s;
        __syncthreads();
    }
}

struct GenPlan {
    uint64_t msg_lens, msg_data, msg_bloom; uint32_t msg_bloom_words, msg_lens_const;
    uint64_t lvl_data, lvl_meta; uint32_t lvl_dict_len; uint8_t lvl_ids[8];
    uint64_t path_lens, path_data, path_bloom; uint32_t path_bloom_words, path_lens_const;
    uint64_t st_data, st_bloom; uint32_t st_bloom_words;
};

__device__ void bloom_add(unsigned long long* words, uint32_t nwords, uint64_t token_hash) {
    if (!nwords) return;
    uint64_t maxbits = (uint64_t)nwords * 64;
    for (int k = 0; k < 6; k++) { uint64_t idx = xxh64_u64(token_hash + k) % maxbits; atomicOr(&words[idx >> 6], 1ull << (idx & 63)); }
}
__device__ __forceinline__ unsigned long long bswap64(unsigned long long x) {
    uint32_t lo = (uint32_t)x, hi = (uint32_t)(x >> 32);
    return ((unsigned long long)__byte_perm(lo, 0, 0x0123) << 32) | __byte_perm(hi, 0, 0x0123);
}

__global__ void __launch_bounds__(256) k_gen_fill(vlscan_gen_config c, uint64_t block_lo, uint32_t nblocks, const GenPlan* __restrict__ plans, uint8_t* __restrict__ arena) {
    __shared__ uint32_t s_off[8192 + 1];
    __shared__ uint32_t s_carry;
    __shared__ uint32_t s_wsum[8];
    for (uint32_t j = blockIdx.x; j < nblocks; j += gridDim.x) {
        const GenPlan& pl = plans[j];
        uint64_t b = block_lo + j;
        uint64_t lo = b * c.rows_per_block, hi = min((unsigned long long)c.total_rows, (unsigned long long)(lo + c.rows_per_block));
        uint32_t rows = (uint32_t)(hi - lo);
        bool hot = gen_rnd(c.seed, b, 0xFFFFFFFFULL, 0) % 1000 < c.hot_block_permille;
        uint8_t buf[192];
        for (int col = 0; col < 2; col++) {
            if (!(c.columns_mask & (col == 0 ? 1 : 4))) continue;
            uint64_t o_lens = col == 0 ? pl.msg_lens : pl.path_lens, o_data = col == 0 ? pl.msg_data : pl.path_data, o_bloom = col == 0 ? pl.msg_bloom : pl.path_bloom;
            uint32_t bw = col == 0 ? pl.msg_bloom_words : pl.path_bloom_words, lconst = col == 0 ? pl.msg_lens_const : pl.path_lens_const;
            if (threadIdx.x == 0) s_carry = 0;
            __syncthreads();
            for (uint32_t base = 0; base < rows; base += blockDim.x) {
                uint32_t i = base + threadIdx.x;
                uint32_t n = 0;
                if (i < rows) n = (uint32_t)(col == 0 ? gen_msg(c, hot, b, i, buf) : gen_path(c, b, i, buf));
                uint32_t incl = n;
#pragma unroll
                for (int d = 1; d < 32; d <<= 1) { uint32_t t = __shfl_up_sync(0xffffffffu, incl, d); if ((threadIdx.x & 31) >= d) incl += t; }
                if ((threadIdx.x & 31) == 31) s_wsum[threadIdx.x >> 5] = incl;
                __syncthreads();
                uint32_t pre = 0; for (uint32_t k = 0; k < (threadIdx.x >> 5); k++) pre += s_wsum[k];
                uint32_t excl = s_carry + pre + incl - n;
                if (i < rows) { s_off[i] = excl; if (lconst == 0xFFFFFFFFu) arena[o_lens + i] = (uint8_t)n; }
                __syncthreads();
                if (threadIdx.x == blockDim.x - 1) s_carry = excl + n;
                __syncthreads();
            }
            if (lconst != 0xFFFFFFFFu && threadIdx.x == 0) arena[o_lens] = (uint8_t)lconst;
            unsigned long long* bloom = (unsigned long long*)(arena + o_bloom);
            for (uint32_t i = threadIdx.x; i < rows; i += blockDim.x) {
                int n = col == 0 ? gen_msg(c, hot, b, i, buf) : gen_path(c, b, i, buf);
                uint8_t* dst = arena + o_data + s_off[i];
                for (int k = 0; k < n; k++) dst[k] = buf[k];
                ascii_tokens(buf, n, [&](const uint8_t* t, uint32_t tl) { bloom_add(bloom, bw, xxh64(t, tl)); });
            }
            __syncthreads();
            for (uint32_t k = threadIdx.x; k < bw; k += blockDim.x) bloom[k] = bswap64(bloom[k]);
            __syncthreads();
        }
        if (c.columns_mask & 2) {
            for (uint32_t i = threadIdx.x; i < rows; i += blockDim.x) arena[pl.lvl_data + i] = pl.lvl_ids[gen_rnd(c.seed, b, i, 5) % 8];
            if (threadIdx.x == 0) {
                uint32_t* offs = (uint32_t*)(arena + pl.lvl_meta); uint8_t* vals = arena + pl.lvl_meta + 4 * (pl.lvl_dict_len + 1);
                uint32_t o = 0;
                for (uint32_t id = 0; id < pl.lvl_dict_len; id++) {
                    for (int v = 0; v < 8; v++) if (pl.lvl_ids[v] == id) { offs[id] = o; o += (uint32_t)put_str(vals + o, D_LEVELS[v]); }
                }
                offs[pl.lvl_dict_len] = o;
            }
        }
        if (c.columns_mask & 8) {
            unsigned long long* bloom = (unsigned long long*)(arena + pl.st_bloom);
            for (uint32_t i = threadIdx.x; i < rows; i += blockDim.x) {
                uint32_t v = D_STATUS[gen_rnd(c.seed, b, i, 7) % 9];
                arena[pl.st_data + 2 * i] = (uint8_t)(v >> 8); arena[pl.st_data + 2 * i + 1] = (uint8_t)v;
                int n = fmt_u64(buf, v);
                bloom_add(bloom, pl.st_bloom_words, xxh64(buf, (uint32_t)n));
            }
            __syncthreads();
            for (uint32_t k = threadIdx.x; k < pl.st_bloom_words; k += blockDim.x) bloom[k] = bswap64(bloom[k]);
        }
        __syncthreads();
    }
}

__global__ void k_gen_poke(uint8_t* arena, const uint64_t* offs, const uint8_t* vals, size_t n) {
    size_t i = (size_t)blockIdx.x * blockDim.x + threadIdx.x;
    if (i < n) arena[offs[i]] = vals[i];
}

}

extern "C" int vlscan_batch_generate(vlscan_ctx* ctx, const vlscan_gen_config* cfgp, uint64_t block_lo, uint64_t block_hi, vlscan_batch** out) {
    *out = nullptr;
    vlscan_batch* bt = new vlscan_batch();
    try {
        vlscan_gen_config c = *cfgp;
        VL_CUDA(cudaSetDevice(ctx->device));
        uint64_t total_blocks = (c.total_rows + c.rows_per_block - 1) / c.rows_per_block;
        if (c.rows_per_block < 64 || c.rows_per_block > 8192) throw BadInput("generator: rows_per_block must be within [64, 8192]");
        if (block_hi > total_blocks || block_lo > block_hi) throw BadInput("generator: block range outside the data set");
        uint32_t nb = (uint32_t)(block_hi - block_lo);
        std::vector<uint32_t> rows(nb);
        for (uint32_t j = 0; j < nb; j++) { uint64_t lo = (block_lo + j) * c.rows_per_block, hi = std::min<uint64_t>(c.total_rows, lo + c.rows_per_block); rows[j] = (uint32_t)(hi - lo); if (rows[j] < 64) throw BadInput("generator: the last block must keep at least 64 rows"); }
        bt->device = ctx->device;
        static const char* const names[4] = {"_msg", "level", "path", "status"};
        int slot_of[4]; bt->nfields = 0;
        for (int k = 0; k < 4; k++) { slot_of[k] = -1; if (c.columns_mask >> k & 1) { slot_of[k] = (int)bt->nfields++; bt->field_names.push_back(names[k]); } }
        if (!bt->nfields) throw BadInput("generator: empty columns_mask");
        if (((c.columns_mask >> 8) & 15) > 12 || (c.columns_mask >> 17) || ((c.columns_mask >> 12) && !(c.columns_mask & 16)))
            throw BadInput("generator: bits 8..11 of columns_mask select a vocabulary entry 1..12, bits 12..16 (interleaved timestamp streams) need bit 4, higher bits must be zero");
        const uint32_t ts_k = (c.columns_mask >> 12) & 31;
        if (ts_k > 16) throw BadInput("generator: at most 2^16 interleaved timestamp streams (bits 12..16 of columns_mask)");
        const uint64_t ts_streams = 1ull << ts_k;
        uint32_t cap = 1; while (cap < c.rows_per_block * 40u) cap <<= 1;
        int grid = std::min<int>(std::max<uint32_t>(nb, 1), ctx->sm_count * 2);
        DevBuf tables, info_d, plans_d;
        tables.ensure((size_t)grid * 3 * cap * 8); info_d.ensure(std::max<size_t>((size_t)nb * sizeof(GenInfo), 16));
        std::vector<GenInfo> info(nb);
        if (nb) {
            k_gen_measure<<<grid, 256, 0, ctx->stream>>>(c, block_lo, nb, info_d.as<GenInfo>(), tables.as<unsigned long long>(), cap - 1);
            ctx->launches++; VL_CUDA(cudaGetLastError());
            VL_CUDA(cudaMemcpyAsync(info.data(), info_d.p, (size_t)nb * sizeof(GenInfo), cudaMemcpyDeviceToHost, ctx->stream));
            VL_CUDA(cudaStreamSynchronize(ctx->stream));
        }
        tables.release();
        std::vector<DevColumn> cols((size_t)nb * bt->nfields); memset(cols.data(), 0, cols.size() * sizeof(DevColumn));
        std::vector<GenPlan> plans(nb); memset(plans.data(), 0, plans.size() * sizeof(GenPlan));
        uint64_t cursor = 16;
        std::vector<DevTimestamps> tsv((c.columns_mask & 16) ? nb : 0);
        if (!tsv.empty()) memset(tsv.data(), 0, tsv.size() * sizeof(DevTimestamps));
        std::vector<uint8_t> ts_varint;
        for (uint64_t u = (ts_streams * VLSCAN_GEN_STEP) << 1; ; u >>= 7) { if (u < 0x80) { ts_varint.push_back((uint8_t)u); break; } ts_varint.push_back((uint8_t)(u | 0x80)); }
        for (uint32_t j = 0; j < nb; j++) {
            const GenInfo& gi = info[j]; GenPlan& pl = plans[j]; uint32_t R = rows[j];
            if (gi.overflow) throw BadInput("generator: token set overflow");
            auto strings_col = [&](int slot, uint32_t bytes, uint32_t minl, uint32_t maxl, uint32_t tokens, uint64_t* o_lens, uint64_t* o_data, uint64_t* o_bloom, uint32_t* bw, uint32_t* lconst) {
                if (maxl >= 256) throw BadInput("generator: row longer than 255 bytes");
                DevColumn& d = cols[(size_t)j * bt->nfields + slot];
                d.kind = COL_VALUES; d.vt = VT_STRING;
                bool cl = R >= 2 && minl == maxl;
                d.lens_type = cl ? 4 : 0; d.lens_const = cl ? maxl : 0; *lconst = cl ? maxl : 0xFFFFFFFFu;
                d.lens_off = *o_lens = arena_reserve(cursor, cl ? 1 : R);
                d.data_off = *o_data = arena_reserve(cursor, bytes); d.data_len = bytes;
                *bw = (tokens * 16 + 63) / 64; d.bloom_words = *bw; d.bloom_off = *o_bloom = arena_reserve(cursor, (uint64_t)*bw * 8);
            };
            if (slot_of[0] >= 0) strings_col(slot_of[0], gi.msg_bytes, gi.msg_minlen, gi.msg_maxlen, gi.msg_tokens, &pl.msg_lens, &pl.msg_data, &pl.msg_bloom, &pl.msg_bloom_words, &pl.msg_lens_const);
            if (slot_of[1] >= 0) {
                std::vector<std::pair<uint32_t, int>> seen;
                for (int v = 0; v < 8; v++) if (gi.level_first[v] != 0xFFFFFFFFu) seen.emplace_back(gi.level_first[v], v);
                std::sort(seen.begin(), seen.end());
                if (seen.size() < 2) throw BadInput("generator: `level` would become a const column in this block");
                memset(pl.lvl_ids, 0xFF, 8);
                uint32_t total = 0; static const uint32_t lvl_len[8] = {5, 4, 4, 5, 5, 5, 5, 4};
                for (size_t id = 0; id < seen.size(); id++) { pl.lvl_ids[seen[id].second] = (uint8_t)id; total += lvl_len[seen[id].second]; }
                pl.lvl_dict_len = (uint32_t)seen.size();
                DevColumn& d = cols[(size_t)j * bt->nfields + slot_of[1]];
                d.kind = COL_VALUES; d.vt = VT_DICT; d.dict_len = (uint8_t)seen.size();
                d.lens_type = 4; d.lens_const = 1;
                d.lens_off = arena_reserve(cursor, 1);
                d.data_off = pl.lvl_data = arena_reserve(cursor, R); d.data_len = R;
                d.bloom_off = arena_reserve(cursor, 0); d.bloom_words = 0;
                d.meta_len = total; d.meta_off = pl.lvl_meta = arena_reserve(cursor, 4 * (seen.size() + 1) + total);
            }
            if (slot_of[2] >= 0) {
                if (gi.path_distinct <= 8) throw BadInput("generator: `path` would become a dict / const column in this block");
                strings_col(slot_of[2], gi.path_bytes, gi.path_minlen, gi.path_maxlen, gi.path_tokens, &pl.path_lens, &pl.path_data, &pl.path_bloom, &pl.path_bloom_words, &pl.path_lens_const);
            }
            if (c.columns_mask & 16) {
                DevTimestamps& t = tsv[j];
                const uint64_t gb = block_lo + j;
                const uint64_t first = (uint64_t)VLSCAN_GEN_T0 + ((gb / ts_streams) * ts_streams * c.rows_per_block + gb % ts_streams) * (uint64_t)VLSCAN_GEN_STEP;
                t.first = (int64_t)first; t.max = (int64_t)(first + (uint64_t)(R - 1) * ts_streams * VLSCAN_GEN_STEP);
                t.mt = MT_DELTA_CONST; t.len = (uint32_t)ts_varint.size(); t.off = arena_reserve(cursor, ts_varint.size());
            }
            if (slot_of[3] >= 0) {
                int present = __builtin_popcount(gi.status_mask);
                if (present <= 8) throw BadInput("generator: `status` would become a dict / const column in this block");
                static const uint32_t st[9] = {200, 201, 204, 301, 400, 404, 500, 502, 503};
                uint32_t mn = 0xFFFFFFFFu, mx = 0; for (int k = 0; k < 9; k++) if (gi.status_mask >> k & 1) { mn = std::min(mn, st[k]); mx = std::max(mx, st[k]); }
                DevColumn& d = cols[(size_t)j * bt->nfields + slot_of[3]];
                d.kind = COL_VALUES; d.vt = VT_UINT16; d.min_value = mn; d.max_value = mx;
                d.lens_type = 4; d.lens_const = 2;
                d.lens_off = arena_reserve(cursor, 1);
                d.data_off = pl.st_data = arena_reserve(cursor, 2ull * R); d.data_len = 2ull * R;
                pl.st_bloom_words = ((uint32_t)present * 16 + 63) / 64; d.bloom_words = pl.st_bloom_words; d.bloom_off = pl.st_bloom = arena_reserve(cursor, (uint64_t)pl.st_bloom_words * 8);
            }
        }
        bt->arena_bytes = cursor + kArenaPad;
        bt->arena.ensure(bt->arena_bytes);
        VL_CUDA(cudaMemsetAsync(bt->arena.p, 0, bt->arena_bytes, ctx->stream));
        plans_d.ensure(std::max<size_t>((size_t)nb * sizeof(GenPlan), 16));
        bt->cols.ensure(std::max<size_t>(cols.size() * sizeof(DevColumn), 16));
        if (nb) {
            VL_CUDA(cudaMemcpyAsync(plans_d.p, plans.data(), (size_t)nb * sizeof(GenPlan), cudaMemcpyHostToDevice, ctx->stream));
            VL_CUDA(cudaMemcpyAsync(bt->cols.p, cols.data(), cols.size() * sizeof(DevColumn), cudaMemcpyHostToDevice, ctx->stream));
            k_gen_fill<<<std::min<int>(nb, ctx->sm_count * 4), 256, 0, ctx->stream>>>(c, block_lo, nb, plans_d.as<GenPlan>(), bt->arena.as<uint8_t>());
            ctx->launches++; VL_CUDA(cudaGetLastError());
            std::vector<std::pair<uint64_t, uint8_t>> pokes;
            for (uint32_t j = 0; j < nb; j++) {
                if (slot_of[1] >= 0) pokes.emplace_back(cols[(size_t)j * bt->nfields + slot_of[1]].lens_off, (uint8_t)1);
                if (slot_of[3] >= 0) pokes.emplace_back(cols[(size_t)j * bt->nfields + slot_of[3]].lens_off, (uint8_t)2);
                if (!tsv.empty()) for (size_t k = 0; k < ts_varint.size(); k++) pokes.emplace_back(tsv[j].off + k, ts_varint[k]);
            }
            if (!pokes.empty()) {
                std::vector<uint64_t> offs(pokes.size()); std::vector<uint8_t> vals(pokes.size());
                for (size_t k = 0; k < pokes.size(); k++) { offs[k] = pokes[k].first; vals[k] = pokes[k].second; }
                DevBuf d_offs, d_vals; d_offs.ensure(offs.size() * 8); d_vals.ensure(vals.size());
                VL_CUDA(cudaMemcpyAsync(d_offs.p, offs.data(), offs.size() * 8, cudaMemcpyHostToDevice, ctx->stream));
                VL_CUDA(cudaMemcpyAsync(d_vals.p, vals.data(), vals.size(), cudaMemcpyHostToDevice, ctx->stream));
                k_gen_poke<<<(unsigned)((offs.size() + 255) / 256), 256, 0, ctx->stream>>>(bt->arena.as<uint8_t>(), d_offs.as<uint64_t>(), d_vals.as<uint8_t>(), offs.size());
                ctx->launches++; VL_CUDA(cudaGetLastError());
                VL_CUDA(cudaStreamSynchronize(ctx->stream));
                d_offs.release(); d_vals.release();
            }
        }
        if (!tsv.empty()) {
            bt->ts.ensure(tsv.size() * sizeof(DevTimestamps));
            VL_CUDA(cudaMemcpyAsync(bt->ts.p, tsv.data(), tsv.size() * sizeof(DevTimestamps), cudaMemcpyHostToDevice, ctx->stream));
            VL_CUDA(cudaStreamSynchronize(ctx->stream));
            bt->has_ts = true;
        }
        bt->note_columns(cols);
        finish_batch_layout(ctx, bt, rows);
        plans_d.release(); info_d.release();
        *out = bt;
        return 0;
    } catch (const CudaFail& e) { set_thread_error(e.msg); ctx->err = e.msg; delete bt; return e.code > 0 ? e.code : 1; }
    catch (const BadInput& e) { set_thread_error(e.msg); ctx->err = e.msg; delete bt; return -1; }
    catch (const std::exception& e) { set_thread_error(e.what()); ctx->err = e.what(); delete bt; return -3; }
}
```

### victorialogs_b200/csrc/vl_zstd.cu

```cuda
#include "vl_zstd.h"

#include <algorithm>
#include <array>
#include <atomic>
#include <chrono>
#include <cstdio>
#include <cstdlib>
#include <cstring>
#include <exception>
#include <thread>

#include "vl_engine.h"
#include "vl_zstd.cuh"
#include "vl_zstd_job.h"

namespace vl {

using namespace zs;

struct ZstdDev {
    DevBuf frames, blocks, bstate, huf_tab, fse_tab, huf_state, fse_state, predef, lits, seqs, frame_err, status, lists;
    bool predef_ready = false;
    cudaStream_t xstream = nullptr;
    std::vector<cudaEvent_t> events;
    cudaEvent_t event(size_t i) {
        while (events.size() <= i) { cudaEvent_t e; VL_CUDA(cudaEventCreateWithFlags(&e, cudaEventDisableTiming)); events.push_back(e); }
        return events[i];
    }
    void* hpin = nullptr; size_t hpin_cap = 0;
    void* ensure_hpin(size_t n) {
        if (n <= hpin_cap) return hpin;
        if (hpin) cudaFreeHost(hpin);
        hpin = nullptr; hpin_cap = 0;
        VL_CUDA(cudaMallocHost(&hpin, n + n / 4 + 4096)); hpin_cap = n + n / 4 + 4096;
        return hpin;
    }
    void release() {
        DevBuf* all[] = {&frames, &blocks, &bstate, &huf_tab, &fse_tab, &huf_state, &fse_state, &predef, &lits, &seqs, &frame_err, &status, &lists};
        for (DevBuf* b : all) b->release();
        for (cudaEvent_t e : events) cudaEventDestroy(e);
        events.clear();
        if (xstream) cudaStreamDestroy(xstream);
        xstream = nullptr;
        if (hpin) cudaFreeHost(hpin);
        hpin = nullptr; hpin_cap = 0;
    }
};

static __global__ void k_pull_words(uint4* __restrict__ dst, const uint4* __restrict__ src, size_t n) {
    for (size_t i = (size_t)blockIdx.x * blockDim.x + threadIdx.x; i < n; i += (size_t)gridDim.x * blockDim.x) dst[i] = src[i];
}
void zstd_dev_free(ZstdDev* d) { if (d) { d->release(); delete d; } }

namespace {
inline unsigned cdiv_u(uint64_t a, uint64_t b) { return (unsigned)((a + b - 1) / b); }
}

struct ZstdJob::Impl : ZstdJobImpl {};

ZstdJob::ZstdJob() : m(new Impl) {}
ZstdJob::~ZstdJob() { delete m; }
bool ZstdJob::empty() const { return m->frames.empty(); }
uint64_t ZstdJob::frames() const { return m->frames.size(); }
uint64_t ZstdJob::blocks() const { return m->blocks.size(); }
uint64_t ZstdJob::compressed_blocks() const { return m->n_compressed; }
uint64_t ZstdJob::sequences() const { return m->n_seqs; }
uint64_t ZstdJob::groups() const { return m->groups.size(); }
void ZstdJob::set_dst(uint32_t id, uint64_t arena_off) { m->frames[id].dst = arena_off; }
void ZstdJob::set_group_hook(std::function<void(uint64_t)> f) { m->group_hook = std::move(f); }

void ZstdJob::add_frame(const uint8_t* f, size_t n, uint64_t zoff, uint64_t* regen, uint32_t* id) {
    ZFrame fr{};
    zwalk::parse_frame_into(m->blocks, (uint32_t)m->frames.size(), f, n, zoff, fr);
    *regen = fr.fcs; *id = (uint32_t)m->frames.size();
    m->commit_frame(fr);
}

size_t ZstdJob::add_bytes_block(const uint8_t* p, size_t n, uint64_t zoff, uint64_t* regen, uint32_t* id) {
    ZFrame fr{};
    const size_t used = zwalk::parse_bytes_block_into(m->blocks, (uint32_t)m->frames.size(), p, n, zoff, fr);
    *regen = fr.fcs; *id = (uint32_t)m->frames.size();
    m->commit_frame(fr);
    return used;
}

void ZstdJob::add_values_blocks(const ZValuesBlock* v, size_t n, int threads, ZValuesInfo* info, size_t* bad, std::string* msg) {
    *bad = SIZE_MAX;
    if (!m->frames.empty()) throw BadInput("BUG: add_values_blocks needs an empty job");
    if (threads > 0) { m->walk_values_blocks(v, n, threads, info, bad, msg); return; }
    uint64_t total_seqs = 0;
    if (!group_scale_env()) {
        ZstdJob dry;
        dry.m->limit_scale = 1u << 20;
        for (size_t i = 0; i < n; i++) {
            try {
                uint64_t r = 0; uint32_t id = 0;
                const size_t c1 = dry.add_bytes_block(v[i].p, v[i].n, v[i].zoff, &r, &id);
                dry.add_bytes_block(v[i].p + c1, v[i].n - c1, v[i].zoff + c1, &r, &id);
            } catch (const BadInput&) { break; }
        }
        total_seqs = dry.m->n_seqs;
    }
    auto taper = [&] { if (!group_scale_env()) m->limit_scale = (m->groups.empty() || m->n_seqs > total_seqs - total_seqs / 12) ? 1 : 4; };
    for (size_t i = 0; i < n; i++) {
        try {
            uint32_t f1 = 0, f2 = 0;
            taper();
            const size_t c1 = add_bytes_block(v[i].p, v[i].n, v[i].zoff, &info[i].lens_len, &f1);
            taper();
            const size_t c2 = add_bytes_block(v[i].p + c1, v[i].n - c1, v[i].zoff + c1, &info[i].data_len, &f2);
            if (c1 + c2 != v[i].n) throw BadInput("unexpected non-empty tail after reading bytes block with strings");
        } catch (const BadInput& e) { *bad = i; *msg = e.msg; return; }
    }
    if (!group_scale_env()) m->limit_scale = 1;
}

void ZstdJob::prepare() { m->prepare(); }

void ZstdJob::digest(uint64_t out[4]) const { m->digest(out); }

void ZstdJob::run(vlscan_ctx* ctx, const uint8_t* zsrc, uint8_t* arena) {
    Impl& J = *m;
    if (J.frames.empty()) return;
    auto now = [] { return std::chrono::duration<double>(std::chrono::steady_clock::now().time_since_epoch()).count(); };
    const double t_prep = now();
    J.prepare();
    const double t_lists = now();
    const std::vector<uint32_t>& lists = J.lists;
    if (!ctx->zdev) ctx->zdev = new ZstdDev;
    ZstdDev& D = *ctx->zdev;
    cudaStream_t st = ctx->stream;
    D.frames.ensure(J.frames.size() * sizeof(ZFrame) + 16); D.blocks.ensure(J.blocks.size() * sizeof(ZBlock) + 16); D.bstate.ensure(J.blocks.size() * sizeof(ZBlockState));
    D.frame_err.ensure(J.frames.size() * 4); D.status.ensure(16); D.lists.ensure(lists.size() * 4 + 16);
    D.huf_tab.ensure(std::max<size_t>((size_t)J.max_huf * Z_HUF_TABLE * 2, 16)); D.huf_state.ensure(std::max<size_t>((size_t)J.max_huf * sizeof(ZSlotState), 16));
    D.fse_tab.ensure(std::max<size_t>((size_t)J.max_fse * Z_FSE_SLOT_BYTES, 16)); D.fse_state.ensure(std::max<size_t>((size_t)J.max_fse * sizeof(ZSlotState), 16));
    const size_t lits_stride = (J.max_lits + 64 + 255) / 256 * 256, seqs_stride = std::max<size_t>(J.max_seqs, 1);
    D.lits.ensure(2 * lits_stride); D.seqs.ensure(2 * seqs_stride * 16);
    if (!D.xstream) VL_CUDA(cudaStreamCreateWithFlags(&D.xstream, cudaStreamNonBlocking));
    if (!D.predef_ready) {
        D.predef.ensure(Z_FSE_SLOT_BYTES);
        k_zstd_predef<<<1, 32, 0, st>>>(D.predef.as<uint8_t>());
        VL_CUDA(cudaFuncSetAttribute(k_seq_decode, cudaFuncAttributeMaxDynamicSharedMemorySize, (int)(Z_SEQ_CTA_LANES * (Z_FSE_SLOT_BYTES + Z_LINEBUF))));
        VL_CUDA(cudaFuncSetAttribute(k_huf_decode, cudaFuncAttributeMaxDynamicSharedMemorySize, (int)(Z_HUF_CTA_BLOCKS * Z_HUF_TABLE * 2)));
        ctx->launches++; VL_CUDA(cudaGetLastError());
        D.predef_ready = true;
    }
    {
        auto up16 = [](size_t n) { return (n + 15) / 16 * 16; };
        const size_t nf = up16(J.frames.size() * sizeof(ZFrame)), nb = up16(J.blocks.size() * sizeof(ZBlock)), nl = up16(lists.size() * 4);
        uint8_t* h = (uint8_t*)D.ensure_hpin(nf + nb + nl + 64);
        const double t_cp = now();
        J.spread_copy(h, J.frames.data(), J.frames.size() * sizeof(ZFrame));
        J.spread_copy(h + nf, J.blocks.data(), J.blocks.size() * sizeof(ZBlock));
        if (!lists.empty()) J.spread_copy(h + nf + nb, lists.data(), lists.size() * 4);
        if (getenv("VLSCAN_DEBUG_TIMING")) fprintf(stderr, "[vlscan zstd] host: work lists of %zu launch groups %.1f ms, %.1f MB of tables to pinned memory %.1f ms (%d threads)\n",
                                                   J.groups.size(), 1e3 * (t_lists - t_prep), (nf + nb + nl) / 1e6, 1e3 * (now() - t_cp), std::max(J.threads, 1));
        k_pull_words<<<296, 256, 0, st>>>(D.frames.as<uint4>(), (const uint4*)h, nf / 16); ctx->launches++;
        k_pull_words<<<296, 256, 0, st>>>(D.blocks.as<uint4>(), (const uint4*)(h + nf), nb / 16); ctx->launches++;
        if (nl) { k_pull_words<<<296, 256, 0, st>>>(D.lists.as<uint4>(), (const uint4*)(h + nf + nb), nl / 16); ctx->launches++; }
        VL_CUDA(cudaGetLastError());
    }
    VL_CUDA(cudaMemsetAsync(D.frame_err.p, 0, J.frames.size() * 4, st));
    VL_CUDA(cudaMemsetAsync(D.status.p, 0, 16, st));
    VL_CUDA(cudaMemsetAsync(D.bstate.p, 0, J.blocks.size() * sizeof(ZBlockState), st));
    ZView V{};
    V.src = zsrc; V.arena = arena; V.frames = D.frames.as<ZFrame>(); V.blocks = D.blocks.as<ZBlock>(); V.bstate = D.bstate.as<ZBlockState>();
    V.huf_tab = D.huf_tab.as<uint16_t>(); V.fse_tab = D.fse_tab.as<uint8_t>(); V.huf_state = D.huf_state.as<ZSlotState>(); V.fse_state = D.fse_state.as<ZSlotState>();
    V.predef = D.predef.as<uint8_t>(); V.lits = D.lits.as<uint8_t>(); V.seqs = D.seqs.as<uint4>(); V.frame_err = D.frame_err.as<unsigned int>();
    V.status = D.status.as<unsigned long long>();
    const uint32_t* L = D.lists.as<uint32_t>();
    const bool dbg = getenv("VLSCAN_DEBUG_TIMING") != nullptr;
    static const char* phase_name[6] = {"huf_build", "huf_decode", "fse_build", "seq_decode", "seq_resolve", "execute"};
    std::vector<std::pair<int, std::pair<cudaEvent_t, cudaEvent_t>>> marks;
    int phase = 0;
    static const bool overlap = [] { const char* e = getenv("VLSCAN_ZSTD_OVERLAP"); return !e || atoi(e) != 0; }();
    cudaStream_t xs = overlap ? D.xstream : st;
    cudaStream_t cur_stream = st;
    auto begin = [&](int p) { phase = p; if (dbg) { cudaEvent_t a, b; cudaEventCreate(&a); cudaEventCreate(&b); cudaEventRecord(a, cur_stream); marks.push_back({p, {a, b}}); } };
    auto launched = [&] { ctx->launches++; VL_CUDA(cudaGetLastError()); if (dbg) cudaEventRecord(marks.back().second.second, cur_stream); };
    VL_CUDA(cudaEventRecord(D.event(0), st)); VL_CUDA(cudaStreamWaitEvent(xs, D.event(0), 0));
    size_t gi = 0;
    for (const Group& g : J.groups) {
        uint32_t nh = g.huf_hi - g.huf_lo, nl = g.lit_hi - g.lit_lo, ns = g.seq_hi - g.seq_lo, nf = g.frame_hi - g.frame_lo;
        if (J.group_hook) {
            uint64_t need = 0;
            for (uint32_t i = J.frames[g.frame_lo].blk_lo; i < J.frames[g.frame_hi - 1].blk_hi; i++) need = std::max<uint64_t>(need, J.blocks[i].src + (J.blocks[i].type == ZB_RLE ? 1 : J.blocks[i].size));
            J.group_hook(need);
        }
        ZView W = V;
        W.lits = V.lits + (gi & 1) * lits_stride; W.seqs = V.seqs + (gi & 1) * seqs_stride;
        cudaEvent_t ev_entropy = D.event(1 + 2 * gi), ev_exec = D.event(2 + 2 * gi);
        cur_stream = st;
        if (gi >= 2) VL_CUDA(cudaStreamWaitEvent(st, D.event(2 + 2 * (gi - 2)), 0));
        if (nh) { begin(0); k_huf_build<<<cdiv_u(nh, 4), 128, 0, st>>>(W, L + g.huf_lo, nh); launched(); }
        if (nl) { begin(1); k_huf_decode<<<cdiv_u(nl, Z_HUF_CTA_BLOCKS), Z_HUF_CTA_BLOCKS * 4, Z_HUF_CTA_BLOCKS * Z_HUF_TABLE * 2, st>>>(W, L + g.lit_lo, nl); launched(); }
        if (ns) {
            begin(2); k_fse_build<<<cdiv_u(ns, 64), 64, 0, st>>>(W, L + g.seq_lo, ns); launched();
            begin(3); k_seq_decode<<<cdiv_u(ns, Z_SEQ_CTA_LANES), 64, Z_SEQ_CTA_LANES * (Z_FSE_SLOT_BYTES + Z_LINEBUF), st>>>(W, L + g.seq_lo, ns); launched();
        }
        VL_CUDA(cudaEventRecord(ev_entropy, st));
        VL_CUDA(cudaStreamWaitEvent(xs, ev_entropy, 0));
        cur_stream = xs;
        begin(4); k_seq_resolve<<<cdiv_u(nf, 64), 64, 0, xs>>>(W, g.frame_lo, nf); launched();
        begin(5); k_execute<<<cdiv_u((uint64_t)nf * 32, Z_EXEC_WARPS * 32), Z_EXEC_WARPS * 32, 0, xs>>>(W, L + g.ord_lo, nf); launched();
        VL_CUDA(cudaEventRecord(ev_exec, xs));
        gi++;
    }
    if (gi) VL_CUDA(cudaStreamWaitEvent(st, D.event(2 + 2 * (gi - 1)), 0));
    cur_stream = st;
    if (dbg) {
        VL_CUDA(cudaStreamSynchronize(xs)); VL_CUDA(cudaStreamSynchronize(st));
        float tot[6] = {0, 0, 0, 0, 0, 0};
        for (auto& mk : marks) { float ms = 0; cudaEventElapsedTime(&ms, mk.second.first, mk.second.second); tot[mk.first] += ms; cudaEventDestroy(mk.second.first); cudaEventDestroy(mk.second.second); }
        fprintf(stderr, "[vlscan zstd] %zu groups:", J.groups.size());
        for (int p = 0; p < 6; p++) fprintf(stderr, " %s %.2f ms", phase_name[p], tot[p]);
        fprintf(stderr, "\n");
    }
    (void)phase;
    J.ran = true;
}

void ZstdJob::check(vlscan_ctx* ctx) {
    if (!m->ran) return;
    unsigned long long stt[2] = {0, 0};
    VL_CUDA(cudaMemcpyAsync(stt, ctx->zdev->status.p, 16, cudaMemcpyDeviceToHost, ctx->stream));
    VL_CUDA(cudaStreamSynchronize(ctx->stream));
    if (!stt[0]) return;
    static const char* what[] = {"", "bad Huffman tree description", "bad Huffman stream", "bad FSE table description", "bad sequences bitstream", "match offset beyond the regenerated data",
                                 "regenerated size differs from the frame content size", "bad literals section"};
    throw BadInput(std::string("cannot decompress block: ") + (stt[0] < 8 ? what[stt[0]] : "corrupted frame") + " (frame " + std::to_string(stt[1] - 1) + " of the batch)");
}

}
```

### victorialogs_b200/csrc/vl_zstd.h

```cpp
#pragma once
#include <stddef.h>
#include <stdint.h>
#include <functional>
#include <string>
#include <vector>

struct vlscan_ctx;

namespace vl {

struct ZstdDev;
void zstd_dev_free(ZstdDev* d);

struct ZstdTimings { float total_ms = 0; };

struct ZValuesBlock { const uint8_t* p; size_t n; uint64_t zoff; };
struct ZValuesInfo { uint64_t lens_len, data_len; };

class ZstdJob {
public:
    ZstdJob();
    ~ZstdJob();
    ZstdJob(const ZstdJob&) = delete;
    ZstdJob& operator=(const ZstdJob&) = delete;
    size_t add_bytes_block(const uint8_t* p, size_t n, uint64_t zoff, uint64_t* regen, uint32_t* id);
    void add_frame(const uint8_t* f, size_t n, uint64_t zoff, uint64_t* regen, uint32_t* id);
    void add_values_blocks(const ZValuesBlock* v, size_t n, int threads, ZValuesInfo* info, size_t* bad, std::string* msg);
    void prepare();
    void digest(uint64_t out[4]) const;
    void set_dst(uint32_t id, uint64_t arena_off);
    bool empty() const;
    uint64_t frames() const;
    uint64_t blocks() const;
    uint64_t compressed_blocks() const;
    uint64_t sequences() const;
    uint64_t groups() const;
    void set_group_hook(std::function<void(uint64_t src_end)> f);
    void run(vlscan_ctx* ctx, const uint8_t* zsrc, uint8_t* arena);
    void check(vlscan_ctx* ctx);
private:
    struct Impl;
    Impl* m;
};

}
```

Baseline: 22.71 billion.

## Start GPU zstd decode before describing columns and overlap copies with it

The decompression region is now laid out at the front of the arena and sized from a host-computed upper bound on the copied bytes, so the zstd decoder can be launched right after the frame headers are walked instead of after every column is described. Only the gaps between decoded frames are zeroed by a new kernel, rather than memsetting the whole arena up front. The on-disk column table upload and the batch layout tables move to the copy stream so they overlap with decoding. It also adds an env-gated timeline profiler. The cost is a more complex bound calculation that throws if the copied part outgrows it.

```diff
diff --git a/victorialogs_b200/csrc/vl_engine.cu b/victorialogs_b200/csrc/vl_engine.cu
--- a/victorialogs_b200/csrc/vl_engine.cu
+++ b/victorialogs_b200/csrc/vl_engine.cu
@@ -93,7 +93,7 @@
 }
 
 namespace vl {
-void finish_batch_layout(vlscan_ctx* ctx, vlscan_batch* b, const std::vector<uint32_t>& rows) {
+void finish_batch_layout(vlscan_ctx* ctx, vlscan_batch* b, const std::vector<uint32_t>& rows, cudaStream_t st) {
     b->nblocks = rows.size();
     b->h_rows = rows;
     b->h_word_off.assign(rows.size() + 1, 0);
@@ -111,28 +111,40 @@
     b->blk_word_off.ensure((rows.size() + 1) * 8);
     b->word_block.ensure(std::max<size_t>(b->nwords * 4, 16));
     b->init_bitmap.ensure(std::max<size_t>(b->nwords * 8, 16));
-    if (!rows.empty()) VL_CUDA(cudaMemcpyAsync(b->blk_rows.p, rows.data(), rows.size() * 4, cudaMemcpyHostToDevice, ctx->stream));
-    VL_CUDA(cudaMemcpyAsync(b->blk_word_off.p, b->h_word_off.data(), (rows.size() + 1) * 8, cudaMemcpyHostToDevice, ctx->stream));
+    if (!rows.empty()) VL_CUDA(cudaMemcpyAsync(b->blk_rows.p, rows.data(), rows.size() * 4, cudaMemcpyHostToDevice, st));
+    VL_CUDA(cudaMemcpyAsync(b->blk_word_off.p, b->h_word_off.data(), (rows.size() + 1) * 8, cudaMemcpyHostToDevice, st));
     if (b->nwords) {
-        VL_CUDA(cudaMemcpyAsync(b->word_block.p, wb.data(), b->nwords * 4, cudaMemcpyHostToDevice, ctx->stream));
-        VL_CUDA(cudaMemcpyAsync(b->init_bitmap.p, init.data(), b->nwords * 8, cudaMemcpyHostToDevice, ctx->stream));
-    }
-    VL_CUDA(cudaStreamSynchronize(ctx->stream));
-}
-}
-
-static uint64_t collect_values_blocks(const vlscan_block* blocks, uint64_t nblocks, std::vector<ZValuesBlock>& zv, const uint8_t* need = nullptr, uint32_t nfields = 0, std::vector<size_t>* at = nullptr) {
+        VL_CUDA(cudaMemcpyAsync(b->word_block.p, wb.data(), b->nwords * 4, cudaMemcpyHostToDevice, st));
+        VL_CUDA(cudaMemcpyAsync(b->init_bitmap.p, init.data(), b->nwords * 8, cudaMemcpyHostToDevice, st));
+    }
+    VL_CUDA(cudaStreamSynchronize(st));
+}
+}
+
+static uint64_t collect_values_blocks(const vlscan_block* blocks, uint64_t nblocks, std::vector<ZValuesBlock>& zv, const uint8_t* need = nullptr, uint32_t nfields = 0,
+                                      std::vector<size_t>* at = nullptr, uint64_t* copied = nullptr) {
     uint64_t zc = 512;
     if (at) at->assign((size_t)nblocks * nfields, SIZE_MAX);
-    for (uint64_t b = 0; b < nblocks; b++)
+    const uint64_t slack = kArenaAlign + kArenaPad;
+    for (uint64_t b = 0; b < nblocks; b++) {
+        if (copied) *copied += blocks[b].timestamps_len + slack;
         for (uint32_t k = 0; k < blocks[b].ncols; k++) {
             const vlscan_column& c = blocks[b].cols[k];
+            if (copied) {
+                if (c.kind == VLSCAN_COL_CONST) *copied += c.const_len + slack;
+                else {
+                    *copied += c.bloom_len + 4 * slack;
+                    if (c.kind == VLSCAN_COL_VALUES && c.value_type == VT_DICT && c.dict_len <= 8) *copied += 4 * (c.dict_len + 1) + (c.dict_len ? c.dict_offsets[c.dict_len] : 0);
+                    if (c.stage == VLSCAN_STAGE_DECODED) *copied += c.lens_items_len + c.data_len;
+                }
+            }
             if (c.kind != VLSCAN_COL_VALUES || c.stage != VLSCAN_STAGE_ONDISK) continue;
             if (need && (c.field >= nfields || !need[b * nfields + c.field])) continue;
             if (at && c.field < nfields && (*at)[b * nfields + c.field] == SIZE_MAX) (*at)[b * nfields + c.field] = zv.size();
             zv.push_back({c.values, (size_t)c.values_len, zc});
             zc += c.values_len;
         }
+    }
     return zc;
 }
 static double now_s() { return std::chrono::duration<double>(std::chrono::steady_clock::now().time_since_epoch()).count(); }
@@ -149,14 +161,12 @@
     std::vector<std::unique_ptr<std::vector<uint8_t>>> owned;
     uint64_t cursor = 16;
     ZstdJob zjob;
-    uint64_t regen_cursor = 0;
-    struct Ondisk { uint64_t col; uint32_t lens_frame, data_frame; uint64_t lens_rel, data_rel; };
-    std::vector<Ondisk> ondisk;
+    bool decoding = false;
+    uint64_t regen_end = 0;
     std::vector<OndiskCol> ocols;
-    struct TsFrame { uint64_t block; uint32_t frame; uint64_t rel; };
-    std::vector<TsFrame> ts_frames;
     std::vector<DevTimestamps> tsv;
-    std::vector<ZValuesBlock> zv; std::vector<ZValuesInfo> zinfo; std::vector<size_t> zv_of; std::vector<uint64_t> ts_zoff; size_t zbad = SIZE_MAX; std::string zmsg;
+    std::vector<ZValuesBlock> zv; std::vector<ZValuesInfo> zinfo; std::vector<size_t> zv_of; std::vector<uint64_t> zv_at; size_t zbad = SIZE_MAX; std::string zmsg;
+    std::vector<uint64_t> ts_zoff, ts_regen, ts_at; size_t ts_bad = SIZE_MAX; std::string ts_msg;
     uint64_t add_piece(const uint8_t* src, uint64_t len) { uint64_t off = arena_reserve(cursor, len); if (len) pieces.push_back({src, len, off}); return off; }
     template <class F> void walk(bool ts, F&& f) {
         for (uint64_t b = 0; b < nblocks; b++) {
@@ -170,10 +180,11 @@
             }
         }
     }
-    void sources(const uint8_t* need, bool ts) {
-        uint64_t zc = collect_values_blocks(blocks, nblocks, zv, need, nfields, &zv_of);
+    void sources(const uint8_t* need, bool ts, DevBuf& region) {
+        uint64_t copied = 0;
+        uint64_t zc = collect_values_blocks(blocks, nblocks, zv, need, nfields, &zv_of, &copied);
         for (const ZValuesBlock& v : zv) if (v.n) io.src.push_back({v.p, v.n, v.zoff});
-        ts_zoff.resize(ts ? nblocks : 0);
+        ts_zoff.assign(ts ? nblocks : 0, 0);
         for (uint64_t b = 0; b < nblocks && ts; b++) {
             const vlscan_block& blk = blocks[b];
             if (blk.ts_marshal_type != MT_ZSTD_NEAREST_DELTA2 && blk.ts_marshal_type != MT_ZSTD_NEAREST_DELTA) continue;
@@ -183,11 +194,50 @@
             zc += blk.timestamps_len;
         }
         if (!io.src.empty()) { ctx->zsrc.ensure(zc + 512); io.send_sources(ctx->zsrc.as<uint8_t>()); }
+        timeline().host("upload: compressed bytes enqueued");
+        timeline().dev("copy stream: compressed bytes landed", ctx->copy_stream);
         zinfo.resize(zv.size());
         const double t_w = now_s();
         if (!zv.empty()) zjob.add_values_blocks(zv.data(), zv.size(), host_threads(), zinfo.data(), &zbad, &zmsg);
+        ts_regen.assign(ts_zoff.size(), 0);
+        for (uint64_t b = 0; b < ts_zoff.size() && ts_bad == SIZE_MAX; b++) {
+            const vlscan_block& blk = blocks[b];
+            if (blk.ts_marshal_type != MT_ZSTD_NEAREST_DELTA2 && blk.ts_marshal_type != MT_ZSTD_NEAREST_DELTA) continue;
+            try {
+                uint32_t id = 0;
+                zjob.add_frame(blk.timestamps, blk.timestamps_len, ts_zoff[b], &ts_regen[b], &id);
+                if (ts_regen[b] > 10ull * blk.rows + 16) throw BadInput("cannot unmarshal timestamps: the decompressed block is larger than its varints can be");
+            } catch (const BadInput& e) { ts_bad = b; ts_msg = e.msg; }
+        }
+        timeline().host("upload: frame headers walked");
         if (dbg) fprintf(stderr, "[vlscan upload] header walk of %zu values blocks on %d host threads: %.1f ms (after %.1f ms of collecting and enqueueing the copies)\n",
                          zv.size(), host_threads(), 1e3 * (now_s() - t_w), 1e3 * (t_w - t_start));
+        if (zv.empty() && ts_regen.empty()) return;
+        zv_at.resize(2 * zv.size());
+        uint32_t id = 0;
+        for (size_t z = 0; z < zv.size(); z++) {
+            zv_at[2 * z] = arena_reserve(cursor, zinfo[z].lens_len + 15); zjob.set_dst(id++, zv_at[2 * z] + 15);
+            zv_at[2 * z + 1] = arena_reserve(cursor, zinfo[z].data_len); zjob.set_dst(id++, zv_at[2 * z + 1]);
+        }
+        ts_at.assign(ts_zoff.size(), 0);
+        for (uint64_t b = 0; b < ts_zoff.size(); b++) {
+            if (blocks[b].ts_marshal_type != MT_ZSTD_NEAREST_DELTA2 && blocks[b].ts_marshal_type != MT_ZSTD_NEAREST_DELTA) continue;
+            ts_at[b] = arena_reserve(cursor, ts_regen[b]); zjob.set_dst(id++, ts_at[b]);
+        }
+        regen_end = cursor;
+        if (zbad != SIZE_MAX || ts_bad != SIZE_MAX || zjob.empty()) return;
+        region.ensure(regen_end + copied + kArenaAlign + kArenaPad);
+        if (getenv("VLSCAN_DEBUG_ARENA_FILL")) {
+            VL_CUDA(cudaMemsetAsync(region.p, 0xFF, region.cap, ctx->stream));
+            cudaEvent_t e = io.events.make();
+            VL_CUDA(cudaEventRecord(e, ctx->stream)); VL_CUDA(cudaStreamWaitEvent(ctx->copy_stream, e, 0));
+        }
+        zjob.set_group_hook([this](uint64_t src_end) { io.wait_sources(ctx->stream, src_end); });
+        zjob.run(ctx, ctx->zsrc.as<uint8_t>(), region.as<uint8_t>());
+        zjob.zero_gaps(ctx, region.as<uint8_t>(), regen_end);
+        timeline().host("upload: decoder enqueued");
+        io.ship_sources(UINT64_MAX);
+        decoding = true;
     }
     template <class F> void header(const vlscan_column& c, size_t i, F&& payload) {
         DevColumn& d = cols[i];
@@ -227,9 +277,7 @@
             if (z >= zbad) throw BadInput(zmsg);
             const uint64_t lens_len = zinfo[z].lens_len, data_len = zinfo[z].data_len;
             if (data_len > 0xFFFFFFFFull) throw BadInput("values block too large");
-            const uint64_t lr = arena_reserve(regen_cursor, lens_len + 15), dr = arena_reserve(regen_cursor, data_len);
-            d.lens_off = lr + 16; d.data_off = dr; d.data_len = data_len;
-            ondisk.push_back({ci, (uint32_t)(2 * z), (uint32_t)(2 * z + 1), lr + 15, dr});
+            d.lens_off = zv_at[2 * z] + 16; d.data_off = zv_at[2 * z + 1]; d.data_len = data_len;
             ocols.push_back({ci, lens_len, blk.rows});
         } else if (c.stage == VLSCAN_STAGE_DECODED) {
             const uint8_t* lens_items = c.lens_items; const uint64_t lens_len = c.lens_items_len, data_len = c.data_len;
@@ -254,12 +302,10 @@
         DevTimestamps& t = tsv[b];
         t.first = blk.min_timestamp; t.max = blk.max_timestamp;
         if (blk.ts_marshal_type == MT_ZSTD_NEAREST_DELTA2 || blk.ts_marshal_type == MT_ZSTD_NEAREST_DELTA) {
-            uint64_t regen = 0; uint32_t id = 0;
-            zjob.add_frame(blk.timestamps, blk.timestamps_len, ts_zoff[b], &regen, &id);
-            if (regen > 10ull * blk.rows + 16) throw BadInput("cannot unmarshal timestamps: the decompressed block is larger than its varints can be");
+            if (b == ts_bad) throw BadInput(ts_msg);
             t.mt = blk.ts_marshal_type == MT_ZSTD_NEAREST_DELTA2 ? MT_NEAREST_DELTA2 : MT_NEAREST_DELTA;
-            t.len = (uint32_t)regen;
-            ts_frames.push_back({b, id, arena_reserve(regen_cursor, regen)});
+            t.len = (uint32_t)ts_regen[b];
+            t.off = ts_at[b];
         } else {
             t.mt = (uint8_t)blk.ts_marshal_type; t.len = (uint32_t)blk.timestamps_len;
             t.off = add_piece(blk.timestamps, blk.timestamps_len);
@@ -267,18 +313,13 @@
     }
 
     uint64_t commit(DevBuf& region, const std::vector<uint64_t>* patch, bool layout) {
-        const uint64_t regen_base = (cursor + kArenaAlign - 1) / kArenaAlign * kArenaAlign;
-        for (const Ondisk& o : ondisk) {
-            DevColumn& d = cols[o.col];
-            d.lens_off += regen_base; d.data_off += regen_base;
-            zjob.set_dst(o.lens_frame, regen_base + o.lens_rel); zjob.set_dst(o.data_frame, regen_base + o.data_rel);
-        }
-        for (const TsFrame& tf : ts_frames) { tsv[tf.block].off = regen_base + tf.rel; zjob.set_dst(tf.frame, regen_base + tf.rel); }
-        const bool have_z = !ondisk.empty() || !ts_frames.empty();
-        if (have_z) cursor = regen_base + regen_cursor;
+        if (zbad != SIZE_MAX || ts_bad != SIZE_MAX) throw BadInput(zbad != SIZE_MAX ? zmsg : ts_msg);
+        const bool have_z = decoding;
+        timeline().host("upload: cells described");
         const uint64_t bytes = cursor + kArenaPad;
         const double t_desc = now_s();
-        region.ensure(bytes);
+        if (!have_z) region.ensure(bytes);
+        else if (bytes > region.cap) throw BadInput("internal: the copied part outgrew its bound");
         const double t_alloc = now_s();
         uint8_t* cols_base = region.as<uint8_t>();
         std::vector<ColPatch> patches;
@@ -293,18 +334,10 @@
             }
         }
         cudaStream_t cs = ctx->copy_stream;
-        cudaEvent_t ev_cleared = io.events.make(), ev_copied = io.events.make();
-        VL_CUDA(cudaMemsetAsync(region.p, 0, bytes, ctx->stream));
-        VL_CUDA(cudaEventRecord(ev_cleared, ctx->stream));
-        VL_CUDA(cudaStreamWaitEvent(cs, ev_cleared, 0));
+        cudaEvent_t ev_copied = io.events.make();
+        const uint64_t copy_lo = have_z ? regen_end : 0;
+        VL_CUDA(cudaMemsetAsync(region.as<uint8_t>() + copy_lo, 0, bytes - copy_lo, cs));
         const double t_h2d = dbg ? now_s() : 0;
-        double t_zrun = 0;
-        if (have_z) {
-            zjob.set_group_hook([&](uint64_t src_end) { io.wait_sources(ctx->stream, src_end); });
-            zjob.run(ctx, ctx->zsrc.as<uint8_t>(), region.as<uint8_t>());
-            io.ship_sources(UINT64_MAX);
-            if (dbg) t_zrun = now_s();
-        }
         io.copy(pieces, region.as<uint8_t>());
         DevBuf& table = patch ? ctx->patch : out->cols;
         const void* entries = patch ? (const void*)patches.data() : (const void*)cols.data();
@@ -318,7 +351,15 @@
             VL_CUDA(cudaMemcpyAsync(out->ts.p, tsv.data(), nblocks * sizeof(DevTimestamps), cudaMemcpyHostToDevice, cs));
             io.h2d += nblocks * sizeof(DevTimestamps);
         }
+        if (have_z) {
+            ctx->zcols.ensure(16 + ocols.size() * sizeof(OndiskCol));
+            VL_CUDA(cudaMemsetAsync(ctx->zcols.p, 0, 16, cs));
+            if (!ocols.empty()) VL_CUDA(cudaMemcpyAsync(ctx->zcols.as<uint8_t>() + 16, ocols.data(), ocols.size() * sizeof(OndiskCol), cudaMemcpyHostToDevice, cs));
+            io.h2d += ocols.size() * sizeof(OndiskCol);
+        }
         VL_CUDA(cudaEventRecord(ev_copied, cs));
+        if (layout) finish_batch_layout(ctx, out, rows, cs);
+        timeline().host("upload: copied part, column table and layout tables landed");
         if (!patches.empty()) {
             VL_CUDA(cudaStreamWaitEvent(ctx->stream, ev_copied, 0));
             k_patch_cols<<<cdiv(patches.size(), 128), 128, 0, ctx->stream>>>(out->cols.as<DevColumn>(), ctx->patch.as<ColPatch>(), (uint32_t)patches.size());
@@ -327,16 +368,14 @@
         const double t_enq = dbg ? now_s() : 0;
         if (have_z) {
             VL_CUDA(cudaStreamWaitEvent(ctx->stream, ev_copied, 0));
-            ctx->zcols.ensure(16 + ocols.size() * sizeof(OndiskCol));
-            VL_CUDA(cudaMemsetAsync(ctx->zcols.p, 0, 16, ctx->stream));
-            VL_CUDA(cudaMemcpyAsync(ctx->zcols.as<uint8_t>() + 16, ocols.data(), ocols.size() * sizeof(OndiskCol), cudaMemcpyHostToDevice, ctx->stream));
             if (!ocols.empty()) {
                 k_finish_ondisk_cols<<<cdiv(ocols.size(), 128), 128, 0, ctx->stream>>>(cols_base, out->cols.as<DevColumn>(), (const OndiskCol*)(ctx->zcols.as<uint8_t>() + 16),
                                                                                          (uint32_t)ocols.size(), ctx->zcols.as<unsigned long long>());
                 launch_check(ctx);
             }
-            io.h2d += ocols.size() * sizeof(OndiskCol);
+            timeline().dev("compute stream: on-disk columns finished", ctx->stream);
             zjob.check(ctx);
+            timeline().host("upload: decode checked");
             unsigned long long cst[2] = {0, 0};
             VL_CUDA(cudaMemcpy(cst, ctx->zcols.p, 16, cudaMemcpyDeviceToHost));
             static const char* what[] = {"", "cannot unmarshal uint64 block type from empty src", "unexpected uint64 block type", "unexpected block length for uint items", "row length does not fit 32 bits"};
@@ -346,12 +385,11 @@
         double t_copy = 0;
         if (dbg) { VL_CUDA(cudaStreamSynchronize(ctx->stream)); t_copy = now_s(); }
         if (nfields) out->note_columns(cols);
-        if (layout) finish_batch_layout(ctx, out, rows);
-        else VL_CUDA(cudaStreamSynchronize(ctx->stream));
+        VL_CUDA(cudaStreamSynchronize(ctx->stream));
         if (dbg) fprintf(stderr, "[vlscan upload] blocks=%llu arena=%.1f MB h2d=%.1f MB pieces=%zu+%zu pinned=%d: describe %.1f ms, alloc %.1f ms, copy %.1f ms (%.1f GB/s), "
-                                 "zstd %llu frames / %llu blocks / %llu sequences: enqueue %.1f ms, decode %.1f ms; layout %.1f ms\n", (unsigned long long)nblocks,
-                         bytes / 1e6, io.h2d / 1e6, pieces.size(), io.src.size(), (int)io.all_pinned, 1e3 * (t_desc - t_start), 1e3 * (t_alloc - t_desc), 1e3 * (t_enq - (t_zrun > 0 ? t_zrun : t_h2d)), io.h2d / 1e9 / std::max(t_copy - t_start, 1e-9),
-                         (unsigned long long)zjob.frames(), (unsigned long long)zjob.compressed_blocks(), (unsigned long long)zjob.sequences(), 1e3 * (t_zrun > 0 ? t_zrun - t_h2d : 0), 1e3 * (t_copy - t_enq), 1e3 * (now_s() - t_copy));
+                                 "zstd %llu frames / %llu blocks / %llu sequences: decode done %.1f ms later; layout %.1f ms\n", (unsigned long long)nblocks,
+                         bytes / 1e6, io.h2d / 1e6, pieces.size(), io.src.size(), (int)io.all_pinned, 1e3 * (t_desc - t_start), 1e3 * (t_alloc - t_desc), 1e3 * (t_enq - t_h2d), io.h2d / 1e9 / std::max(t_copy - t_start, 1e-9),
+                         (unsigned long long)zjob.frames(), (unsigned long long)zjob.compressed_blocks(), (unsigned long long)zjob.sequences(), 1e3 * (t_copy - t_enq), 1e3 * (now_s() - t_copy));
         if (layout) io.h2d += out->nwords * 12 + nblocks * 12;
         if (stats) stats->h2d_bytes += io.h2d;
         return bytes;
@@ -376,7 +414,7 @@
     try {
         switch (mode) {
         case UP_FULL:
-            u.sources(nullptr, true);
+            u.sources(nullptr, true, out->arena);
             u.walk(true, [&](const vlscan_block& blk, const vlscan_column& c, size_t i) { u.header(c, i, [&] { u.values(blk, c, i); }); });
             out->arena_bytes = u.commit(out->arena, nullptr, true);
             out->harena_bytes = 0;
@@ -392,7 +430,7 @@
             out->harena_bytes = u.commit(out->harena, nullptr, true);
             break;
         case UP_VALUES:
-            u.sources(need, true);
+            u.sources(need, true, out->arena);
             u.walk(true, [&](const vlscan_block& blk, const vlscan_column& c, size_t i) {
                 if (c.kind != VLSCAN_COL_VALUES) return;
                 u.cols[i].values_state = need[i] ? VALUES_STAGED : VALUES_ABSENT;
@@ -402,7 +440,8 @@
             break;
         case UP_LATE: {
             std::vector<uint64_t> staged;
-            u.sources(need, false);
+            if (out->late_used == out->late.size()) out->late.emplace_back();
+            u.sources(need, false, out->late[out->late_used]);
             u.walk(false, [&](const vlscan_block& blk, const vlscan_column& c, size_t i) {
                 if (c.kind != VLSCAN_COL_VALUES || !need[i]) return;
                 if (u.cols[i].values_state == VALUES_STAGED) throw BadInput("duplicate column for one field in a block");
@@ -410,7 +449,6 @@
                 u.values(blk, c, i);
                 staged.push_back(i);
             });
-            if (out->late_used == out->late.size()) out->late.emplace_back();
             u.commit(out->late[out->late_used], &staged, false);
             out->late_used++;
             *zframes += u.zjob.frames();
@@ -1165,6 +1203,7 @@
     ctx->recycle = nullptr;
     b->field_names.clear(); b->slot_vt_mask.clear();
     uint64_t launches0 = ctx->launches;
+    timeline().start(ctx->stream);
     std::vector<char> need_bloom(nfields, 0), in_prog(nfields, 0);
     {
         const Program& P = prog->p;
@@ -1219,8 +1258,12 @@
             }
         });
     } else rc = guarded(ctx, [&] { do_upload(ctx, field_names, field_name_lens, nfields, blocks, nblocks, b, stats, &need_bloom); });
+    timeline().dev("compute stream: scan starts", ctx->stream);
     if (!rc) rc = vlscan_scan_resident(ctx, prog, b, nullptr);
+    timeline().dev("compute stream: scan ends", ctx->stream);
     if (!rc) rc = vlscan_fetch_results(ctx, out_bitmap_words, out_match_counts, stats);
+    timeline().host("results fetched");
+    timeline().print();
     if (!rc && stats) {
         rc = guarded(ctx, [&] { read_stats(ctx, stats, true); stats->blocks += b->nblocks; stats->rows += b->rows; stats->gpu_launches += ctx->launches - launches0; });
     }
diff --git a/victorialogs_b200/csrc/vl_engine.h b/victorialogs_b200/csrc/vl_engine.h
--- a/victorialogs_b200/csrc/vl_engine.h
+++ b/victorialogs_b200/csrc/vl_engine.h
@@ -2,6 +2,9 @@
 #include <cuda_runtime.h>
 #include <stdint.h>
 #include <algorithm>
+#include <chrono>
+#include <cstdio>
+#include <cstdlib>
 #include <string>
 #include <vector>
 #include "../../include/vlscan.h"
@@ -34,6 +37,41 @@
 };
 
 
+
+struct Timeline {
+    struct Mark { std::string name; cudaEvent_t ev; double host; };
+    bool on = false;
+    cudaEvent_t t0 = nullptr; double h0 = 0;
+    std::vector<Mark> marks;
+    static double now() { return std::chrono::duration<double>(std::chrono::steady_clock::now().time_since_epoch()).count(); }
+    void start(cudaStream_t s) {
+        marks.clear();
+        on = getenv("VLSCAN_TIMELINE") != nullptr;
+        if (!on) return;
+        if (!t0) cudaEventCreate(&t0);
+        cudaEventRecord(t0, s); h0 = now();
+    }
+    void host(const std::string& name) { if (on) marks.push_back({name, nullptr, now()}); }
+    void dev(const std::string& name, cudaStream_t s) {
+        if (!on) return;
+        cudaEvent_t e; cudaEventCreate(&e); cudaEventRecord(e, s); marks.push_back({name, e, 0});
+    }
+    void print() {
+        if (!on) return;
+        on = false;
+        cudaDeviceSynchronize();
+        std::vector<std::pair<double, std::string>> v;
+        for (Mark& m : marks) {
+            double t = (m.host - h0) * 1e3;
+            if (m.ev) { float ms = 0; cudaEventElapsedTime(&ms, t0, m.ev); t = ms; cudaEventDestroy(m.ev); }
+            v.push_back({t, m.name});
+        }
+        marks.clear();
+        std::stable_sort(v.begin(), v.end(), [](const auto& a, const auto& b) { return a.first < b.first; });
+        for (auto& x : v) fprintf(stderr, "[vlscan timeline] %8.2f ms  %s\n", x.first, x.second.c_str());
+    }
+};
+inline Timeline& timeline() { static Timeline t; return t; }
 
 static const size_t kArenaAlign = 16;
 static const size_t kArenaPad = 32;
@@ -134,7 +172,7 @@
 };
 
 namespace vl {
-void finish_batch_layout(vlscan_ctx* ctx, vlscan_batch* b, const std::vector<uint32_t>& rows);
+void finish_batch_layout(vlscan_ctx* ctx, vlscan_batch* b, const std::vector<uint32_t>& rows, cudaStream_t st);
 
 const uint32_t* row_offsets(vlscan_ctx* ctx, const BatchView& B, int slot, const uint32_t* list, const uint32_t* wc, unsigned long long* stats, int wc_slot);
 
diff --git a/victorialogs_b200/csrc/vl_gen.cu b/victorialogs_b200/csrc/vl_gen.cu
--- a/victorialogs_b200/csrc/vl_gen.cu
+++ b/victorialogs_b200/csrc/vl_gen.cu
@@ -339,7 +339,7 @@
             bt->has_ts = true;
         }
         bt->note_columns(cols);
-        finish_batch_layout(ctx, bt, rows);
+        finish_batch_layout(ctx, bt, rows, ctx->stream);
         plans_d.release(); info_d.release();
         *out = bt;
         return 0;
diff --git a/victorialogs_b200/csrc/vl_zstd.cu b/victorialogs_b200/csrc/vl_zstd.cu
--- a/victorialogs_b200/csrc/vl_zstd.cu
+++ b/victorialogs_b200/csrc/vl_zstd.cu
@@ -49,6 +49,12 @@
 
 static __global__ void k_pull_words(uint4* __restrict__ dst, const uint4* __restrict__ src, size_t n) {
     for (size_t i = (size_t)blockIdx.x * blockDim.x + threadIdx.x; i < n; i += (size_t)gridDim.x * blockDim.x) dst[i] = src[i];
+}
+static __global__ void k_zero_gaps(uint8_t* __restrict__ arena, const ZFrame* __restrict__ fr, uint32_t n, uint64_t end) {
+    for (uint32_t f = blockIdx.x * blockDim.x + threadIdx.x; f <= n; f += gridDim.x * blockDim.x) {
+        const uint64_t lo = f ? fr[f - 1].dst + fr[f - 1].fcs : 0, hi = f < n ? fr[f].dst : end;
+        for (uint64_t i = lo; i < hi; i++) arena[i] = 0;
+    }
 }
 void zstd_dev_free(ZstdDev* d) { if (d) { d->release(); delete d; } }
 
@@ -158,6 +164,7 @@
         k_pull_words<<<296, 256, 0, st>>>(D.frames.as<uint4>(), (const uint4*)h, nf / 16); ctx->launches++;
         k_pull_words<<<296, 256, 0, st>>>(D.blocks.as<uint4>(), (const uint4*)(h + nf), nb / 16); ctx->launches++;
         if (nl) { k_pull_words<<<296, 256, 0, st>>>(D.lists.as<uint4>(), (const uint4*)(h + nf + nb), nl / 16); ctx->launches++; }
+        timeline().host("decoder: work lists and tables enqueued");
         VL_CUDA(cudaGetLastError());
     }
     VL_CUDA(cudaMemsetAsync(D.frame_err.p, 0, J.frames.size() * 4, st));
@@ -187,6 +194,7 @@
             for (uint32_t i = J.frames[g.frame_lo].blk_lo; i < J.frames[g.frame_hi - 1].blk_hi; i++) need = std::max<uint64_t>(need, J.blocks[i].src + (J.blocks[i].type == ZB_RLE ? 1 : J.blocks[i].size));
             J.group_hook(need);
         }
+        timeline().dev("group " + std::to_string(gi) + ": entropy kernels start (its bytes landed)", st);
         ZView W = V;
         W.lits = V.lits + (gi & 1) * lits_stride; W.seqs = V.seqs + (gi & 1) * seqs_stride;
         cudaEvent_t ev_entropy = D.event(1 + 2 * gi), ev_exec = D.event(2 + 2 * gi);
@@ -199,11 +207,13 @@
             begin(3); k_seq_decode<<<cdiv_u(ns, Z_SEQ_CTA_LANES), 64, Z_SEQ_CTA_LANES * (Z_FSE_SLOT_BYTES + Z_LINEBUF), st>>>(W, L + g.seq_lo, ns); launched();
         }
         VL_CUDA(cudaEventRecord(ev_entropy, st));
+        timeline().dev("group " + std::to_string(gi) + ": entropy kernels end", st);
         VL_CUDA(cudaStreamWaitEvent(xs, ev_entropy, 0));
         cur_stream = xs;
         begin(4); k_seq_resolve<<<cdiv_u(nf, 64), 64, 0, xs>>>(W, g.frame_lo, nf); launched();
         begin(5); k_execute<<<cdiv_u((uint64_t)nf * 32, Z_EXEC_WARPS * 32), Z_EXEC_WARPS * 32, 0, xs>>>(W, L + g.ord_lo, nf); launched();
         VL_CUDA(cudaEventRecord(ev_exec, xs));
+        timeline().dev("group " + std::to_string(gi) + ": execute end", xs);
         gi++;
     }
     if (gi) VL_CUDA(cudaStreamWaitEvent(st, D.event(2 + 2 * (gi - 1)), 0));
@@ -220,6 +230,13 @@
     J.ran = true;
 }
 
+void ZstdJob::zero_gaps(vlscan_ctx* ctx, uint8_t* arena, uint64_t end) {
+    if (!m->ran) return;
+    const uint32_t n = (uint32_t)m->frames.size();
+    k_zero_gaps<<<cdiv_u((uint64_t)n + 1, 256), 256, 0, ctx->stream>>>(arena, ctx->zdev->frames.as<ZFrame>(), n, end);
+    ctx->launches++; VL_CUDA(cudaGetLastError());
+}
+
 void ZstdJob::check(vlscan_ctx* ctx) {
     if (!m->ran) return;
     unsigned long long stt[2] = {0, 0};
diff --git a/victorialogs_b200/csrc/vl_zstd.h b/victorialogs_b200/csrc/vl_zstd.h
--- a/victorialogs_b200/csrc/vl_zstd.h
+++ b/victorialogs_b200/csrc/vl_zstd.h
@@ -37,6 +37,7 @@
     uint64_t groups() const;
     void set_group_hook(std::function<void(uint64_t src_end)> f);
     void run(vlscan_ctx* ctx, const uint8_t* zsrc, uint8_t* arena);
+    void zero_gaps(vlscan_ctx* ctx, uint8_t* arena, uint64_t end);
     void check(vlscan_ctx* ctx);
 private:
     struct Impl;
```

Result: no change. 22.70 billion (median of 6 runs) (-0.0%).
